# silencht/SG-SLAM

Hardware: AMD Instinct MI355X
Metric: tracked frames/sec (640x480 RGB-D) (higher is better)
Workload: dtype u8/f32(bf16x3 matrix products)/f64

## Files before the change

### include/sgx_debug.h

```cpp
#ifndef SGX_DEBUG_H
#define SGX_DEBUG_H
#include "sgx.h"
#ifdef __cplusplus
extern "C" {
#endif

int sgx_orb_debug_level_geometry(const sgx_orb *h, int level, int32_t *w, int32_t *hgt, int32_t *stride);
int sgx_orb_debug_set_unfused_pyramid(int on);
int sgx_orb_debug_read_level(sgx_orb *h, int frame, int level, uint8_t *dst );
int sgx_orb_debug_read_candidates(sgx_orb *h, int frame, int level, int32_t *x, int32_t *y, int32_t *score, int cap, int *n);
int sgx_debug_flow_affine_batch_dev(int batch, int cap, const sgx_keypoint *d_keys, const int32_t *d_n, const float *d_A, const float *d_shift, const float *d_boxes,
                                    int max_boxes, float *d_prev_xy, void *stream);
int sgx_pose_opt_debug_set_threads(int threads_per_frame);
int sgx_ba_debug_last_plan(int32_t plan[4]);
int sgx_ba_debug_set_init(int mode);
int sgx_ba_debug_set_jobs(int host);
int sgx_ba_debug_set_solver(int mode);
int sgx_det_debug_read_blob(sgx_det *h, const char *blob_name, int image, float *dst, int cap, int *n);
int sgx_flow_debug_read_level(sgx_flow *h, int slot, int frame, int level, uint8_t *img);
int sgx_flow_debug_level_size(const sgx_flow *h, int level, int32_t *w, int32_t *hgt);
int sgx_pnp_debug_betas(int which, const double *L, const double *rho, double *betas);
int sgx_debug_corun_bf16(int blocks, int iters, int launches, void *stream);
int sgx_det_debug_detection_output(sgx_det *h, const float *loc, const float *conf, int batch, sgx_det_result *results);
int sgx_det_debug_continued(sgx_det *h, int *count);
int sgx_det_debug_set_fusion(int on);
int sgx_det_debug_set_irb(int on);
int sgx_det_debug_set_block_fusion(int on);
int sgx_det_debug_set_gemm(int mode);
int sgx_det_debug_set_legacy_kernels(int on);
int sgx_det_debug_time_ops(sgx_det *h, const uint8_t *d_img, int pitch, int batch, int reps, float *ms, int cap, int *nops);
int sgx_det_debug_run_step(sgx_det *h, const uint8_t *d_img, int pitch, int batch, int step, int reps, void *stream);
int sgx_orb_debug_run_octree(sgx_orb *h, int level, const uint32_t *packed, int n, uint32_t *out_sel, int cap, int *nsel);

#ifdef __cplusplus
}
#endif
#endif
```

### sg_slam_amd/capi.py

```python
import ctypes as C
import numpy as np

KP_DTYPE = np.dtype([('x', 'f4'), ('y', 'f4'), ('size', 'f4'), ('angle', 'f4'), ('response', 'f4'),
                     ('octave', 'i4'), ('class_id', 'i4')])


class SgxError(RuntimeError):
    pass


class Camera(C.Structure):
    _fields_ = [('fx', C.c_float), ('fy', C.c_float), ('cx', C.c_float), ('cy', C.c_float), ('bf', C.c_float),
                ('min_x', C.c_float), ('max_x', C.c_float), ('min_y', C.c_float), ('max_y', C.c_float)]


class BaProblem(C.Structure):
    _fields_ = [('n_poses', C.c_int32), ('n_points', C.c_int32), ('n_edges', C.c_int32), ('poses', C.c_void_p), ('pose_fixed', C.c_void_p),
                ('points', C.c_void_p), ('edge_pose', C.c_void_p), ('edge_point', C.c_void_p), ('edge_obs', C.c_void_p), ('edge_info', C.c_void_p)]


class BaStats(C.Structure):
    _fields_ = [('iterations_first', C.c_int32), ('iterations_second', C.c_int32), ('free_poses', C.c_int32), ('reserved', C.c_int32),
                ('chi2_first', C.c_double), ('chi2_second', C.c_double)]


SGX_DET_MAX = 100


class Detection(C.Structure):
    _fields_ = [(k, C.c_float) for k in ('label', 'score', 'xmin', 'ymin', 'xmax', 'ymax')]


class Object2D(C.Structure):
    _fields_ = [('id', C.c_int32)] + [(k, C.c_float) for k in ('prob', 'x', 'y', 'w', 'h')]


class DetResult(C.Structure):
    _fields_ = [('n_raw', C.c_int32), ('raw', Detection * SGX_DET_MAX), ('n_objects', C.c_int32), ('objects', Object2D * SGX_DET_MAX),
                ('have_dynamic_for_mapping', C.c_int32), ('have_dynamic_for_rm_feature', C.c_int32),
                ('n_map_boxes', C.c_int32), ('map_boxes', Object2D * SGX_DET_MAX), ('n_rm_boxes', C.c_int32), ('rm_boxes', Object2D * SGX_DET_MAX)]


class FlowConfig(C.Structure):
    _fields_ = [('width', C.c_int32), ('height', C.c_int32), ('max_batch', C.c_int32), ('win_size', C.c_int32), ('max_level', C.c_int32),
                ('max_count', C.c_int32), ('epsilon', C.c_double)]


class TrackerConfig(C.Structure):
    _fields_ = [('streams', C.c_int32), ('width', C.c_int32), ('height', C.c_int32), ('nfeatures', C.c_int32), ('scale_factor', C.c_float), ('nlevels', C.c_int32),
                ('ini_th_fast', C.c_int32), ('min_th_fast', C.c_int32), ('cam', Camera), ('depth_map_factor', C.c_float), ('th_projection', C.c_float),
                ('local_map', C.c_int32), ('dynamic_mask', C.c_int32), ('max_boxes', C.c_int32), ('pipelined', C.c_int32)]


class OrbConfig(C.Structure):
    _fields_ = [('nfeatures', C.c_int32), ('scale_factor', C.c_float), ('nlevels', C.c_int32),
                ('ini_th_fast', C.c_int32), ('min_th_fast', C.c_int32), ('width', C.c_int32),
                ('height', C.c_int32), ('max_batch', C.c_int32)]


SYMBOLS = [
    'sgx_version', 'sgx_status_string', 'sgx_orb_create', 'sgx_orb_destroy', 'sgx_orb_keypoint_capacity', 'sgx_orb_get_tables',
    'sgx_orb_extract_batch_dev', 'sgx_orb_extract', 'sgx_orb_last_status', 'sgx_profile_enable', 'sgx_profile_num_classes', 'sgx_profile_class_name',
    'sgx_profile_read', 'sgx_match_project_frame_batch_dev', 'sgx_match_project_frame', 'sgx_match_project_local_batch_dev',
    'sgx_match_project_local', 'sgx_frame_stereo_from_rgbd_batch_dev', 'sgx_frame_unproject_batch_dev', 'sgx_frame_make_map_points_batch_dev',
    'sgx_frame_merge_matches_batch_dev', 'sgx_pose_optimization_batch_dev', 'sgx_pose_optimization', 'sgx_frame_motion_model_batch_dev',
    'sgx_local_bundle_adjustment', 'sgx_bundle_adjustment', 'sgx_det_create', 'sgx_det_destroy', 'sgx_det_info', 'sgx_det_detect',
    'sgx_det_detect_batch_dev', 'sgx_det_forward_batch_dev', 'sgx_frame_compact_keys_batch_dev', 'sgx_frame_gray_from_color_batch_dev',
    'sgx_det_gemm_mode', 'sgx_det_plan_step', 'sgx_dynamic_mask_batch_dev', 'sgx_tracker_create', 'sgx_tracker_destroy',
    'sgx_tracker_keypoint_capacity', 'sgx_tracker_record_bytes', 'sgx_tracker_set_initial_pose', 'sgx_tracker_step_dev', 'sgx_tracker_host_buffers',
    'sgx_tracker_step_host', 'sgx_tracker_wait_inputs', 'sgx_tracker_sync', 'sgx_tracker_read', 'sgx_tracker_snapshot_pose_dev',
    'sgx_tracker_snapshot_boxes_dev', 'sgx_tracker_pack_records_dev', 'sgx_tracker_frame_dev', 'sgx_tracker_extractor', 'sgx_flow_create',
    'sgx_dist_unique_id', 'sgx_dist_create', 'sgx_dist_destroy', 'sgx_dist_world', 'sgx_dist_gather_records',
    'sgx_flow_destroy', 'sgx_flow_reset', 'sgx_flow_levels', 'sgx_flow_lk_batch_dev', 'sgx_flow_lk', 'sgx_fundamental_ransac_batch_dev',
    'sgx_find_fundamental_mat', 'sgx_hamming_matrix', 'sgx_hamming_matrix_dev', 'sgx_match_search_for_triangulation', 'sgx_match_search_by_bow',
    'sgx_match_search_by_bow_kf', 'sgx_match_fuse_search', 'sgx_match_project_keyframe', 'sgx_match_fuse_search_sim3',
    'sgx_triangulate_new_map_points', 'sgx_mappoint_update_normal_and_depth', 'sgx_mappoint_distinctive_descriptors', 'sgx_sim3_solver_create',
    'sgx_sim3_solver_set_ransac_parameters', 'sgx_sim3_solver_iterate', 'sgx_sim3_solver_get_estimate', 'sgx_sim3_solver_destroy',
    'sgx_match_search_for_initialization', 'sgx_voc_load', 'sgx_voc_create', 'sgx_voc_info', 'sgx_voc_destroy', 'sgx_voc_transform',
    'sgx_voc_transform_batch_dev', 'sgx_voc_score', 'sgx_match_project_sim3', 'sgx_match_search_by_sim3', 'sgx_optimize_sim3',
    'sgx_optimize_essential_graph', 'sgx_correct_map_points', 'sgx_undistort_points', 'sgx_frame_undistort_stereo_rgbd_batch_dev', 'sgx_frame_image_bounds',
    'sgx_tracker_set_distortion', 'sgx_tracker_frame_keys_un_dev', 'sgx_pnp_solver_create', 'sgx_pnp_solver_set_ransac_parameters', 'sgx_pnp_solver_iterate',
    'sgx_pnp_solver_get_estimate', 'sgx_pnp_solver_destroy', 'sgx_pnp_batch_create', 'sgx_pnp_batch_set_dev', 'sgx_pnp_batch_iterate_dev', 'sgx_pnp_batch_destroy',
]
TAP_SYMBOLS = [
    'sgx_orb_debug_level_geometry', 'sgx_orb_debug_set_unfused_pyramid', 'sgx_orb_debug_read_level', 'sgx_orb_debug_read_candidates',
    'sgx_orb_debug_run_octree', 'sgx_pose_opt_debug_set_threads', 'sgx_ba_debug_set_solver', 'sgx_ba_debug_set_jobs', 'sgx_ba_debug_set_init', 'sgx_ba_debug_last_plan', 'sgx_det_debug_read_blob',
    'sgx_det_debug_detection_output', 'sgx_det_debug_continued', 'sgx_debug_flow_affine_batch_dev', 'sgx_det_debug_set_fusion', 'sgx_det_debug_set_legacy_kernels',
    'sgx_det_debug_set_block_fusion', 'sgx_det_debug_set_irb', 'sgx_det_debug_set_gemm', 'sgx_det_debug_time_ops', 'sgx_det_debug_run_step', 'sgx_flow_debug_read_level',
    'sgx_flow_debug_level_size', 'sgx_debug_corun_bf16', 'sgx_pnp_debug_betas',
]


def _vp(x):
    if x is None:
        return None
    if isinstance(x, int):
        return C.c_void_p(x)
    if hasattr(x, 'data_ptr'):
        return C.c_void_p(x.data_ptr())
    return x.ctypes.data_as(C.c_void_p)


class SgxLib:
    def __init__(self, path):
        self.path = path
        self.dll = C.CDLL(path)
        d = self.dll
        d.sgx_version.restype = C.c_char_p
        d.sgx_status_string.restype = C.c_char_p
        d.sgx_status_string.argtypes = [C.c_int]
        d.sgx_orb_create.argtypes = [C.POINTER(OrbConfig), C.POINTER(C.c_void_p)]
        d.sgx_orb_destroy.argtypes = [C.c_void_p]
        d.sgx_orb_destroy.restype = None
        d.sgx_orb_keypoint_capacity.argtypes = [C.c_void_p]
        d.sgx_orb_get_tables.argtypes = [C.c_void_p] + [C.c_void_p] * 5
        d.sgx_orb_extract_batch_dev.argtypes = [C.c_void_p, C.c_void_p, C.c_int, C.c_int, C.c_void_p, C.c_void_p,
                                                C.c_void_p, C.c_int, C.c_void_p]
        d.sgx_orb_extract.argtypes = [C.c_void_p, C.c_void_p, C.c_int, C.c_void_p, C.c_void_p, C.c_int, C.POINTER(C.c_int)]
        d.sgx_orb_last_status.argtypes = [C.c_void_p, C.c_void_p]

        d.sgx_profile_enable.argtypes = [C.c_int]
        d.sgx_profile_class_name.restype = C.c_char_p
        d.sgx_profile_class_name.argtypes = [C.c_int]
        d.sgx_profile_read.argtypes = [C.c_void_p, C.c_void_p, C.c_int]

        vp = C.c_void_p
        d.sgx_match_project_frame_batch_dev.argtypes = [C.c_int, C.c_int] + [vp] * 13 + [C.POINTER(Camera), vp, C.c_int, C.c_float, C.c_int, C.c_int, vp, vp, vp]
        d.sgx_match_project_frame.argtypes = [C.c_int] + [vp] * 4 + [C.c_int] + [vp] * 7 + [C.POINTER(Camera), vp, C.c_int, C.c_float, C.c_int, C.c_int, vp, vp]
        d.sgx_frame_stereo_from_rgbd_batch_dev.argtypes = [C.c_int, C.c_int, vp, vp, vp, C.c_int, C.c_int, C.c_float, C.c_float, vp, vp, vp]
        d.sgx_frame_unproject_batch_dev.argtypes = [C.c_int, C.c_int, vp, vp, vp, vp, C.POINTER(Camera), vp, vp, vp]
        d.sgx_pose_optimization_batch_dev.argtypes = [C.c_int, C.c_int, vp, vp, vp, vp, vp, vp, C.c_int, vp, C.c_int, C.POINTER(Camera), vp, vp, vp, vp]
        d.sgx_pose_optimization.argtypes = [C.c_int, vp, vp, vp, vp, vp, C.c_int, C.POINTER(Camera), vp, vp, vp]
        d.sgx_frame_motion_model_batch_dev.argtypes = [C.c_int, vp, vp, vp, vp, vp]
        d.sgx_local_bundle_adjustment.argtypes = [C.POINTER(BaProblem), C.POINTER(Camera), vp, vp, C.POINTER(BaStats)]
        d.sgx_bundle_adjustment.argtypes = [C.POINTER(BaProblem), C.POINTER(Camera), C.c_int, vp, C.c_int, C.POINTER(BaStats)]
        d.sgx_det_create.argtypes = [C.c_char_p, vp, C.c_size_t, C.c_int, C.c_int, C.c_int, C.c_float, C.c_float, C.POINTER(vp)]
        d.sgx_det_destroy.argtypes = [vp]; d.sgx_det_destroy.restype = None
        d.sgx_det_info.argtypes = [vp, C.POINTER(C.c_int32), C.POINTER(C.c_int32), C.POINTER(C.c_int32), C.POINTER(C.c_double)]
        d.sgx_det_detect.argtypes = [vp, vp, C.c_int, C.c_int, C.POINTER(DetResult)]
        d.sgx_det_detect_batch_dev.argtypes = [vp, vp, C.c_int, C.c_int, vp, vp, vp, C.c_int, vp, vp]
        d.sgx_det_forward_batch_dev.argtypes = [vp, vp, C.c_int, C.c_int, C.POINTER(vp), C.POINTER(vp), vp]
        d.sgx_det_gemm_mode.argtypes = [vp]
        d.sgx_tracker_create.argtypes = [C.POINTER(TrackerConfig), vp, C.POINTER(vp)]
        d.sgx_tracker_destroy.argtypes = [vp]; d.sgx_tracker_destroy.restype = None
        d.sgx_tracker_keypoint_capacity.argtypes = [vp]
        d.sgx_tracker_record_bytes.argtypes = [vp]
        d.sgx_tracker_set_initial_pose.argtypes = [vp, vp]
        d.sgx_tracker_step_dev.argtypes = [vp, vp, C.c_int, vp, vp, C.c_int, vp]
        d.sgx_tracker_host_buffers.argtypes = [vp, C.c_int, C.POINTER(vp), C.POINTER(C.c_int), C.POINTER(vp)]
        d.sgx_tracker_step_host.argtypes = [vp, C.c_int, C.c_int]
        d.sgx_tracker_sync.argtypes = [vp]
        d.sgx_tracker_wait_inputs.argtypes = [vp, C.c_int]
        d.sgx_tracker_read.argtypes = [vp] * 10
        d.sgx_tracker_snapshot_pose_dev.argtypes = [vp, vp]
        d.sgx_tracker_snapshot_boxes_dev.argtypes = [vp, C.c_int, vp, vp]
        d.sgx_tracker_pack_records_dev.argtypes = [vp, vp, vp]
        d.sgx_dist_unique_id.argtypes = [vp]
        d.sgx_dist_create.argtypes = [vp, C.c_int, C.c_int, C.POINTER(vp)]
        d.sgx_dist_destroy.argtypes = [vp]; d.sgx_dist_destroy.restype = None
        d.sgx_dist_world.argtypes = [vp, C.POINTER(C.c_int32), C.POINTER(C.c_int32)]
        d.sgx_dist_gather_records.argtypes = [vp, vp, C.c_size_t, vp, C.c_int, vp]
        d.sgx_tracker_frame_dev.argtypes = [vp] + [C.POINTER(vp)] * 6
        d.sgx_tracker_extractor.argtypes = [vp]; d.sgx_tracker_extractor.restype = vp
        d.sgx_det_plan_step.argtypes = [vp, C.c_int, C.c_char_p, C.c_int]
        d.sgx_dynamic_mask_batch_dev.argtypes = [C.c_int, C.c_int, vp, vp, vp, vp, vp, vp, C.c_int, vp, vp]
        d.sgx_frame_gray_from_color_batch_dev.argtypes = [C.c_int, C.c_int, C.c_int, vp, C.c_int, C.c_int, C.c_int, vp, C.c_int, vp]
        d.sgx_frame_compact_keys_batch_dev.argtypes = [C.c_int, C.c_int, vp, vp, vp, vp, vp, C.c_int, vp, vp, vp, vp]
        d.sgx_match_project_local.argtypes = [C.c_int] + [vp] * 5 + [C.c_int] + [vp] * 7 + [C.POINTER(Camera), vp, C.c_int, C.c_float, C.c_float, C.c_float, C.c_float, vp, vp, vp]
        d.sgx_match_project_local_batch_dev.argtypes = [C.c_int, C.c_int] + [vp] * 6 + [C.c_int] + [vp] * 8 + [C.POINTER(Camera), vp, C.c_int, C.c_float, C.c_float, C.c_float, C.c_float, vp, vp, vp, vp]
        d.sgx_undistort_points.argtypes = [C.c_int, vp, vp, vp, C.c_int, vp]
        d.sgx_frame_undistort_stereo_rgbd_batch_dev.argtypes = [C.c_int, C.c_int, vp, vp, vp, C.c_int, C.POINTER(Camera), vp, C.c_int, C.c_int, C.c_float, vp, vp, vp, vp]
        d.sgx_frame_image_bounds.argtypes = [C.c_int, C.c_int, vp, vp, C.c_int, C.POINTER(Camera)]
        d.sgx_tracker_set_distortion.argtypes = [vp, vp, C.c_int, C.POINTER(Camera)]
        d.sgx_tracker_frame_keys_un_dev.argtypes = [vp, C.POINTER(vp)]
        d.sgx_frame_make_map_points_batch_dev.argtypes = [C.c_int, C.c_int, C.c_int] + [vp] * 7 + [C.c_int] + [vp] * 7
        d.sgx_frame_merge_matches_batch_dev.argtypes = [C.c_int, C.c_int] + [vp] * 10
        d.sgx_flow_create.argtypes = [C.POINTER(FlowConfig), C.POINTER(vp)]
        d.sgx_flow_destroy.argtypes = [vp]; d.sgx_flow_destroy.restype = None
        d.sgx_flow_reset.argtypes = [vp]
        d.sgx_flow_levels.argtypes = [vp]
        d.sgx_flow_lk_batch_dev.argtypes = [vp, vp, C.c_int, C.c_int, vp, vp, C.c_int, vp, vp, C.POINTER(C.c_int32), vp]
        d.sgx_flow_lk.argtypes = [vp, vp, vp, C.c_int, vp, C.c_int, vp, vp]
        d.sgx_fundamental_ransac_batch_dev.argtypes = [C.c_int, C.c_int] + [vp] * 6 + [C.c_int, C.c_double, C.c_double, vp, vp, vp, vp]
        d.sgx_find_fundamental_mat.argtypes = [vp, vp, C.c_int, C.c_double, C.c_double, vp, vp, vp]
        d.sgx_hamming_matrix.argtypes = [vp, C.c_int, vp, C.c_int, vp]
        d.sgx_optimize_essential_graph.argtypes = [C.c_int, vp, vp, C.c_int, vp, vp, vp, C.c_int, C.c_int, vp, vp]
        d.sgx_correct_map_points.argtypes = [C.c_int, vp, vp, C.c_int, vp, vp, vp]
        d.sgx_optimize_sim3.argtypes = [C.c_int] + [vp] * 9 + [C.c_float, C.c_int, vp, vp, vp]
        d.sgx_match_project_keyframe.argtypes = [C.c_int] + [vp] * 4 + [C.c_int] + [vp] * 6 + [C.POINTER(Camera), vp, C.c_int, C.c_float, C.c_float, C.c_int, C.c_int, vp, vp]
        d.sgx_match_search_by_bow.argtypes = [C.c_int] + [vp] * 4 + [C.c_int] + [vp] * 3 + [C.c_float, C.c_int, vp, vp]
        d.sgx_match_fuse_search_sim3.argtypes = [C.c_int, vp, vp, vp, C.c_int] + [vp] * 6 + [vp, vp, C.c_int, C.c_float, C.c_float, vp, vp, vp]
        d.sgx_match_project_sim3.argtypes = [C.c_int, vp, vp, vp, vp, C.c_int] + [vp] * 6 + [vp, vp, C.c_int, C.c_float, C.c_int, vp, vp]
        d.sgx_match_search_by_sim3.argtypes = ([C.c_int] + [vp] * 8) * 2 + [vp, vp, C.c_int, C.c_float, C.c_float, vp, vp, C.c_float, vp, vp]
        d.sgx_match_search_for_initialization.argtypes = [C.c_int, vp, vp, C.c_int, vp, vp, vp, C.c_int, C.c_float, C.c_int, vp, vp, vp]
        d.sgx_sim3_solver_create.argtypes = [C.c_int] + [vp] * 6 + [C.c_int, C.c_uint, vp]
        d.sgx_sim3_solver_set_ransac_parameters.argtypes = [vp, C.c_double, C.c_int, C.c_int]
        d.sgx_sim3_solver_iterate.argtypes = [vp, C.c_int] + [vp] * 7
        d.sgx_sim3_solver_get_estimate.argtypes = [vp] * 5
        d.sgx_sim3_solver_destroy.argtypes = [vp]; d.sgx_sim3_solver_destroy.restype = None
        d.sgx_pnp_solver_create.argtypes = [C.c_int] + [vp] * 4 + [C.c_uint, vp]
        d.sgx_pnp_solver_set_ransac_parameters.argtypes = [vp, C.c_double, C.c_int, C.c_int, C.c_int, C.c_float, C.c_float]
        d.sgx_pnp_solver_iterate.argtypes = [vp, C.c_int] + [vp] * 7
        d.sgx_pnp_solver_get_estimate.argtypes = [vp] * 6
        d.sgx_pnp_solver_destroy.argtypes = [vp]; d.sgx_pnp_solver_destroy.restype = None
        d.sgx_pnp_batch_create.argtypes = [C.c_int, C.c_int, vp]
        d.sgx_pnp_batch_set_dev.argtypes = [vp, C.c_int] + [vp] * 8
        d.sgx_pnp_batch_iterate_dev.argtypes = [vp, C.c_int, vp, C.c_int, vp, vp, vp, vp]
        d.sgx_pnp_batch_destroy.argtypes = [vp]; d.sgx_pnp_batch_destroy.restype = None
        d.sgx_mappoint_update_normal_and_depth.argtypes = [C.c_int] + [vp] * 6 + [C.c_int, vp, vp, vp]
        d.sgx_mappoint_distinctive_descriptors.argtypes = [C.c_int, vp, vp, vp, vp]
        d.sgx_triangulate_new_map_points.argtypes = [C.c_int, vp] + [C.c_int] + [vp] * 5 + [C.c_int] + [vp] * 5 + [vp, vp, vp, C.c_int, vp, vp, vp]
        d.sgx_voc_load.argtypes = [C.c_char_p, vp]
        d.sgx_voc_create.argtypes = [C.c_int] * 5 + [vp] * 5
        d.sgx_voc_info.argtypes = [vp] * 7
        d.sgx_voc_destroy.argtypes = [vp]; d.sgx_voc_destroy.restype = None
        d.sgx_voc_transform.argtypes = [vp, C.c_int, vp, C.c_int, vp, vp, vp, vp, vp]
        d.sgx_voc_transform_batch_dev.argtypes = [vp, vp, C.c_size_t, vp, C.c_int, C.c_int, C.c_int, vp, vp, vp, vp]
        d.sgx_voc_score.argtypes = [vp, C.c_int, vp, vp, C.c_int, vp, vp, vp]
        d.sgx_match_search_by_bow_kf.argtypes = [C.c_int] + [vp] * 4 + [C.c_int] + [vp] * 4 + [C.c_float, C.c_int, vp, vp]
        d.sgx_match_fuse_search.argtypes = [C.c_int] + [vp] * 4 + [C.c_int] + [vp] * 6 + [C.POINTER(Camera), vp, vp, C.c_int, C.c_float, C.c_float, vp, vp, vp]
        d.sgx_hamming_matrix_dev.argtypes = [vp, C.c_int, vp, C.c_int, vp, vp]
        d.sgx_match_search_for_triangulation.argtypes = [C.c_int] + [vp] * 6 + [C.c_int] + [vp] * 6 + [vp, C.POINTER(Camera), vp, vp, C.c_int, C.c_int, C.c_int, vp, vp]

        self.has_taps = hasattr(d, 'sgx_det_debug_read_blob')
        if self.has_taps:
            d.sgx_orb_debug_level_geometry.argtypes = [C.c_void_p, C.c_int] + [C.POINTER(C.c_int32)] * 3
            d.sgx_orb_debug_read_level.argtypes = [C.c_void_p, C.c_int, C.c_int, C.c_void_p]
            d.sgx_orb_debug_read_candidates.argtypes = [C.c_void_p, C.c_int, C.c_int, C.c_void_p, C.c_void_p, C.c_void_p, C.c_int, C.POINTER(C.c_int)]
            d.sgx_orb_debug_run_octree.argtypes = [C.c_void_p, C.c_int, C.c_void_p, C.c_int, C.c_void_p, C.c_int, C.POINTER(C.c_int)]
            d.sgx_orb_debug_set_unfused_pyramid.argtypes = [C.c_int]
            d.sgx_pose_opt_debug_set_threads.argtypes = [C.c_int]
            d.sgx_ba_debug_set_solver.argtypes = [C.c_int]
            d.sgx_ba_debug_set_jobs.argtypes = [C.c_int]
            d.sgx_ba_debug_set_init.argtypes = [C.c_int]
            d.sgx_ba_debug_last_plan.argtypes = [C.c_void_p]
            d.sgx_det_debug_detection_output.argtypes = [vp, vp, vp, C.c_int, C.POINTER(DetResult)]
            d.sgx_det_debug_continued.argtypes = [vp, C.POINTER(C.c_int)]
            d.sgx_det_debug_read_blob.argtypes = [vp, C.c_char_p, C.c_int, vp, C.c_int, C.POINTER(C.c_int)]
            for nm in ('fusion', 'legacy_kernels', 'block_fusion', 'irb', 'gemm'):
                getattr(d, 'sgx_det_debug_set_' + nm).argtypes = [C.c_int]
            d.sgx_det_debug_time_ops.argtypes = [vp, vp, C.c_int, C.c_int, C.c_int, vp, C.c_int, C.POINTER(C.c_int)]
            d.sgx_det_debug_run_step.argtypes = [vp, vp, C.c_int, C.c_int, C.c_int, C.c_int, vp]
            d.sgx_debug_flow_affine_batch_dev.argtypes = [C.c_int, C.c_int, vp, vp, vp, vp, vp, C.c_int, vp, vp]
            d.sgx_flow_debug_read_level.argtypes = [vp, C.c_int, C.c_int, C.c_int, vp]
            d.sgx_debug_corun_bf16.argtypes = [C.c_int, C.c_int, C.c_int, vp]
            d.sgx_pnp_debug_betas.argtypes = [C.c_int, vp, vp, vp]
            d.sgx_flow_debug_level_size.argtypes = [vp, C.c_int, C.POINTER(C.c_int32), C.POINTER(C.c_int32)]

    def tap(self, name):
        if not self.has_taps:
            raise SgxError(f'{name}: {self.path} is the product build and has no test taps; use tests/taps/libsgx_taps.so (make -C sg_slam_amd/csrc taps)')
        return getattr(self.dll, name)

    def version(self):
        return self.dll.sgx_version().decode()

    def check(self, rc, what=''):
        if rc != 0:
            raise SgxError(f'{what}: {self.dll.sgx_status_string(rc).decode()} ({rc})')

    def profile_enable(self, on=True):
        self.check(self.dll.sgx_profile_enable(int(on)))

    def profile_read(self, reset=True):
        n = self.dll.sgx_profile_num_classes()
        ms = np.zeros(n, 'f4'); cnt = np.zeros(n, 'i4')
        self.check(self.dll.sgx_profile_read(_vp(ms), _vp(cnt), int(reset)), 'sgx_profile_read')
        return {self.dll.sgx_profile_class_name(k).decode(): (float(ms[k]), int(cnt[k])) for k in range(n)}
```

### sg_slam_amd/csrc/sgx_flow.cpp

```cpp
#include "sgx_flow_kernels.h"
#include "sgx_prof.h"
#include "sgx_stage.h"
#include "../../include/sgx.h"
#ifdef SGX_DEBUG_TAPS
#include "../../include/sgx_debug.h"
#endif
#include <stdio.h>
#include <stdlib.h>
#include <string.h>
#include <new>
#include <vector>


struct sgx_flow {
    sgx_flow_config cfg;
    SgxLkGeom g;
    uint8_t *img[2] = { nullptr, nullptr };
    int cur = 0;
    int prev_batch = 0;
};

extern "C" int sgx_flow_create(const sgx_flow_config *cfg, sgx_flow **out)
{
    if (!cfg || !out) return SGX_ERR_INVALID;
    *out = nullptr;
    if (cfg->width < 1 || cfg->height < 1 || cfg->max_batch < 1 || cfg->max_count < 0 || !(cfg->epsilon >= 0)) return SGX_ERR_INVALID;
    if (cfg->win_size != SGX_LK_WIN || cfg->max_level < 0 || cfg->max_level >= SGX_LK_MAXL) return SGX_ERR_UNSUPPORTED;
    if (cfg->width <= 1 || cfg->height <= 1) return SGX_ERR_UNSUPPORTED;
    { const unsigned long long qw = (unsigned long long)((cfg->width + 3) >> 2); if (qw * qw * (unsigned long long)cfg->height >= (1ull << 32)) return SGX_ERR_UNSUPPORTED; }
    sgx_flow *h = new (std::nothrow) sgx_flow();
    if (!h) return SGX_ERR_NOMEM;
    h->cfg = *cfg;
    SgxLkGeom &g = h->g;
    memset(&g, 0, sizeof g);
    int w = cfg->width, hh = cfg->height; unsigned io = 0;
    for (int l = 0;; l++) {
        g.w[l] = w; g.h[l] = hh; g.pitch[l] = (w + 3) & ~3; g.ioff[l] = io;
        io += (unsigned)g.pitch[l] * (unsigned)hh;
        g.nl = l + 1;
        if (l == cfg->max_level) break;
        const int nw = (w + 1) / 2, nh = (hh + 1) / 2;
        if (nw <= cfg->win_size || nh <= cfg->win_size) break;
        w = nw; hh = nh;
    }
    g.img_stride = (io + 15u + 64u) & ~15u;
    for (int s = 0; s < 2; s++)
        if (hipMalloc((void **)&h->img[s], (size_t)g.img_stride * cfg->max_batch) != hipSuccess) { sgx_flow_destroy(h); return SGX_ERR_NOMEM; }
    *out = h;
    return SGX_OK;
}

extern "C" void sgx_flow_destroy(sgx_flow *h)
{
    if (!h) return;
    for (int s = 0; s < 2; s++) if (h->img[s]) (void)hipFree(h->img[s]);
    delete h;
}

extern "C" int sgx_flow_reset(sgx_flow *h) { if (!h) return SGX_ERR_INVALID; h->prev_batch = 0; return SGX_OK; }
extern "C" int sgx_flow_levels(const sgx_flow *h) { return h ? h->g.nl : SGX_ERR_INVALID; }

static int build_pyramid(sgx_flow *h, int slot, const uint8_t *d_gray, int pitch, int batch, sgx_stream_t st)
{
    const SgxLkGeom &g = h->g;
    uint8_t *base = h->img[slot];
    sgx_prof_begin(SGX_K_LK_PYR, st);
    auto magic = [](int d) -> unsigned { return d <= 1 ? 0u : (unsigned)((0x100000000ull + (unsigned)d - 1) / (unsigned)d); };
    SGX_LAUNCH(k_lk_copy, dim3(((g.pitch[0] >> 2) * g.h[0] + 255) / 256, batch), dim3(256), st, d_gray, g.w[0], g.h[0], pitch, base, g.pitch[0], g.img_stride, magic(g.pitch[0] >> 2));
    for (int l = 1; l < g.nl; l++)
        SGX_LAUNCH(k_lk_pyrdown, dim3(((g.pitch[l] >> 2) * g.h[l] + 255) / 256, batch), dim3(256), st, (const uint8_t *)(base + g.ioff[l - 1]), g.w[l - 1], g.h[l - 1], g.pitch[l - 1],
                   g.img_stride, base + g.ioff[l], g.w[l], g.h[l], g.pitch[l], g.img_stride, magic(g.pitch[l] >> 2));
    sgx_prof_end(SGX_K_LK_PYR, st);
    SGX_CHECK_HIP(hipGetLastError());
    return SGX_OK;
}

static int track(sgx_flow *h, int cur_slot, int prev_slot, int batch, const sgx_keypoint *d_keys, const int32_t *d_n, int cap, float *d_prev_xy, uint8_t *d_status, sgx_stream_t st)
{
    SgxLkArgs A;
    A.cur_img = h->img[cur_slot]; A.prev_img = h->img[prev_slot];
    A.keys = (const uint8_t *)d_keys; A.n = d_n; A.cap = cap; A.prev_xy = d_prev_xy; A.status = d_status;
    A.max_count = h->cfg.max_count > 100 ? 100 : h->cfg.max_count;
    double eps = h->cfg.epsilon > 10. ? 10. : h->cfg.epsilon;
    A.eps2 = eps * eps; A.min_eig = (float)1e-4;
    sgx_prof_begin(SGX_K_LK_TRACK, st);
    static const int kpw = sgx_getenv("SGX_LK_KPW") ? atoi(sgx_getenv("SGX_LK_KPW")) : 2;
    A.batch = batch; A.kblocks = (cap + 4 * kpw - 1) / (4 * kpw);
#ifdef SGX_DEBUG_TAPS
    if (kpw == 4) { auto kfn = k_lk_trackN<4>; SGX_LAUNCH(kfn, dim3((unsigned)A.kblocks * (unsigned)batch), dim3(256), st, h->g, A); }
    else if (kpw != 2) { A.kblocks = (cap + 3) / 4; SGX_LAUNCH(k_lk_track, dim3((unsigned)A.kblocks * (unsigned)batch), dim3(256), st, h->g, A); }
    else
#endif
    { auto kfn = k_lk_trackN<2>; SGX_LAUNCH(kfn, dim3((unsigned)A.kblocks * (unsigned)batch), dim3(256), st, h->g, A); }
    sgx_prof_end(SGX_K_LK_TRACK, st);
    SGX_CHECK_HIP(hipGetLastError());
    return SGX_OK;
}

extern "C" int sgx_flow_lk_batch_dev(sgx_flow *h, const uint8_t *d_gray, int pitch, int batch, const sgx_keypoint *d_keys, const int32_t *d_n, int cap,
                                     float *d_prev_xy, uint8_t *d_status, int32_t *have_prev, void *stream)
{
    if (!h || !d_gray || batch < 1 || batch > h->cfg.max_batch || pitch < h->cfg.width) return SGX_ERR_INVALID;
    if ((pitch & 3) || ((uintptr_t)d_gray & 3)) return SGX_ERR_INVALID;
    sgx_stream_t st = (sgx_stream_t)stream;
    const int cur = h->cur, prev = cur ^ 1;
    const bool tracked = h->prev_batch == batch;
    if (tracked && (!d_keys || !d_n || !d_prev_xy || cap < 1)) return SGX_ERR_INVALID;
    int rc = build_pyramid(h, cur, d_gray, pitch, batch, st);
    if (rc != SGX_OK) return rc;
    if (tracked) { rc = track(h, cur, prev, batch, d_keys, d_n, cap, d_prev_xy, d_status, st); if (rc != SGX_OK) return rc; }
    if (have_prev) *have_prev = tracked ? 1 : 0;
    h->cur = prev; h->prev_batch = batch;
    return SGX_OK;
}

extern "C" int sgx_flow_lk(sgx_flow *h, const uint8_t *gray_from, const uint8_t *gray_to, int stride, const float *pts, int n, float *next_pts, uint8_t *status)
{
    if (!h || !gray_from || !gray_to || stride < h->cfg.width || n < 0 || (n > 0 && (!pts || !next_pts))) return SGX_ERR_INVALID;
    if (n == 0) return SGX_OK;
    const int W = h->cfg.width, H = h->cfg.height, P = (W + 3) & ~3;
    std::vector<uint8_t> pack((size_t)P * H * 2, 0);
    for (int y = 0; y < H; y++) { memcpy(&pack[(size_t)y * P], gray_to + (size_t)y * stride, (size_t)W); memcpy(&pack[(size_t)(H + y) * P], gray_from + (size_t)y * stride, (size_t)W); }
    std::vector<sgx_keypoint> kp((size_t)n);
    for (int i = 0; i < n; i++) { memset(&kp[(size_t)i], 0, sizeof(sgx_keypoint)); kp[(size_t)i].x = pts[2 * i]; kp[(size_t)i].y = pts[2 * i + 1]; }
    SgxStaged dI, dK, dN, dO, dS;
    int rc;
    if ((rc = dI.put(0, pack.data(), pack.size())) != SGX_OK || (rc = dK.put(1, kp.data(), kp.size() * sizeof(sgx_keypoint))) != SGX_OK ||
        (rc = dN.put(2, &n, sizeof n)) != SGX_OK || (rc = dO.put(3, nullptr, (size_t)n * 8)) != SGX_OK || (rc = dS.put(4, nullptr, (size_t)n)) != SGX_OK) return rc;
    const int keep_cur = h->cur, keep_prev = h->prev_batch;
    if ((rc = build_pyramid(h, 1, (const uint8_t *)dI.p, P, 1, 0)) != SGX_OK) return rc;
    if ((rc = build_pyramid(h, 0, (const uint8_t *)dI.p + (size_t)P * H, P, 1, 0)) != SGX_OK) return rc;
    if ((rc = track(h, 0, 1, 1, (const sgx_keypoint *)dK.p, (const int32_t *)dN.p, n, (float *)dO.p, (uint8_t *)dS.p, 0)) != SGX_OK) return rc;
    SGX_CHECK_HIP(hipMemcpy(next_pts, dO.p, (size_t)n * 8, hipMemcpyDeviceToHost));
    if (status) SGX_CHECK_HIP(hipMemcpy(status, dS.p, (size_t)n, hipMemcpyDeviceToHost));
    h->cur = keep_cur; h->prev_batch = 0; (void)keep_prev;
    return SGX_OK;
}

SGX_TAP int sgx_flow_debug_read_level(sgx_flow *h, int slot, int frame, int level, uint8_t *img )
{
    if (!h || slot < 0 || slot > 1 || frame < 0 || frame >= h->cfg.max_batch || level < 0 || level >= h->g.nl) return SGX_ERR_INVALID;
    const SgxLkGeom &g = h->g;
    SGX_CHECK_HIP(hipDeviceSynchronize());
    if (!img) return SGX_ERR_INVALID;
    {
        std::vector<uint8_t> t((size_t)g.pitch[level] * g.h[level]);
        SGX_CHECK_HIP(hipMemcpy(t.data(), h->img[slot] + (size_t)frame * g.img_stride + g.ioff[level], t.size(), hipMemcpyDeviceToHost));
        for (int y = 0; y < g.h[level]; y++) memcpy(img + (size_t)y * g.w[level], &t[(size_t)y * g.pitch[level]], (size_t)g.w[level]);
    }
    return SGX_OK;
}
SGX_TAP int sgx_flow_debug_level_size(const sgx_flow *h, int level, int32_t *w, int32_t *hh)
{
    if (!h || level < 0 || level >= h->g.nl || !w || !hh) return SGX_ERR_INVALID;
    *w = h->g.w[level]; *hh = h->g.h[level];
    return SGX_OK;
}

#if defined(SGX_DEBUG_TAPS) && !defined(SGX_EMU)
typedef float sgx_dbg_f16v __attribute__((ext_vector_type(16)));
typedef __bf16 sgx_dbg_bf8 __attribute__((ext_vector_type(8)));
SGX_KERNEL_OCC(256, 2) k_dbg_corun_bf16(float *o, int iters)
{
    const uint32_t x = threadIdx.x * 2654435761u + blockIdx.x, y = x ^ 0x9e3779b9u;
    sgx_dbg_f16v acc = {0}; sgx_dbg_bf8 a, b;
    for (int i = 0; i < 8; i++) { a[i] = (__bf16)(float)((x >> i) & 7); b[i] = (__bf16)(float)((y >> i) & 3); }
    for (int i = 0; i < iters; i++) acc = __builtin_amdgcn_mfma_f32_32x32x16_bf16(a, b, acc, 0, 0, 0);
    float s = 0.f; for (int i = 0; i < 16; i++) s += acc[i];
    o[(blockIdx.x & 1023) * 256 + threadIdx.x] = s;
}
#endif
SGX_TAP int sgx_debug_corun_bf16(int blocks, int iters, int launches, void *stream)
{
#if defined(SGX_DEBUG_TAPS) && !defined(SGX_EMU)
    static float *sink = nullptr;
    if (blocks < 1 || iters < 1 || launches < 1) return SGX_ERR_INVALID;
    if (!sink) SGX_CHECK_HIP(hipMalloc((void **)&sink, 1024 * 256 * sizeof(float)));
    for (int l = 0; l < launches; l++) SGX_LAUNCH(k_dbg_corun_bf16, dim3((unsigned)blocks), dim3(256), (sgx_stream_t)stream, sink, iters);
    SGX_CHECK_HIP(hipGetLastError());
    return SGX_OK;
#else
    (void)blocks; (void)iters; (void)launches; (void)stream;
    return SGX_ERR_UNSUPPORTED;
#endif
}

extern "C" int sgx_fundamental_ransac_batch_dev(int batch, int cap, const sgx_keypoint *d_keys, const int32_t *d_n, const float *d_prev_xy,
                                                const int32_t *d_pre_have_dynamic, const float *d_pre_boxes, const int32_t *d_pre_nboxes, int max_boxes,
                                                double threshold, double confidence, double *d_F, int32_t *d_ok, int32_t *d_stats, void *stream)
{
    if (batch < 1 || cap < 1 || !d_keys || !d_n || !d_prev_xy || !d_F || !d_ok || max_boxes < 0) return SGX_ERR_INVALID;
    if (cap > SGX_FM_MAXPTS) return SGX_ERR_UNSUPPORTED;
    SgxFmArgs A;
    A.keys = (const uint8_t *)d_keys; A.n = d_n; A.cap = cap; A.prev_xy = d_prev_xy;
    A.pre_have = d_pre_have_dynamic; A.pre_boxes = d_pre_boxes; A.pre_nboxes = d_pre_nboxes; A.max_boxes = max_boxes;
    if (threshold <= 0) threshold = 3;
    if (confidence < DBL_EPSILON || confidence > 1 - DBL_EPSILON) confidence = 0.99;
    A.threshold = threshold; A.confidence = confidence; A.max_iters = 1000;
    A.F = d_F; A.ok = d_ok; A.stats = d_stats;
    const size_t lds = (size_t)cap * 16 + 1024 + (((size_t)cap + 15) & ~(size_t)15);
    sgx_prof_begin(SGX_K_FM_RANSAC, (sgx_stream_t)stream);
    SGX_LAUNCH_DYN(k_fm_ransac, dim3(batch), dim3(256), lds, (sgx_stream_t)stream, A);
    sgx_prof_end(SGX_K_FM_RANSAC, (sgx_stream_t)stream);
    SGX_CHECK_HIP(hipGetLastError());
    return SGX_OK;
}

extern "C" int sgx_find_fundamental_mat(const float *pts1, const float *pts2, int n, double threshold, double confidence, double *F, int32_t *ok, int32_t *stats)
{
    if (n < 0 || (n > 0 && (!pts1 || !pts2)) || !F || !ok) return SGX_ERR_INVALID;
    if (n > SGX_FM_MAXPTS) return SGX_ERR_UNSUPPORTED;
    const int cap = n > 0 ? n : 1;
    std::vector<sgx_keypoint> kp((size_t)cap);
    memset(kp.data(), 0, kp.size() * sizeof(sgx_keypoint));
    for (int i = 0; i < n; i++) { kp[(size_t)i].x = pts1[2 * i]; kp[(size_t)i].y = pts1[2 * i + 1]; }
    SgxStaged dK, dN, dP, dF, dO, dS;
    int rc;
    if ((rc = dK.put(0, kp.data(), kp.size() * sizeof(sgx_keypoint))) != SGX_OK || (rc = dN.put(1, &n, sizeof n)) != SGX_OK ||
        (rc = dP.put(2, n ? pts2 : nullptr, (size_t)cap * 8)) != SGX_OK || (rc = dF.put(3, nullptr, 72)) != SGX_OK || (rc = dO.put(4, nullptr, 4)) != SGX_OK ||
        (rc = dS.put(5, nullptr, 16)) != SGX_OK) return rc;
    rc = sgx_fundamental_ransac_batch_dev(1, cap, (const sgx_keypoint *)dK.p, (const int32_t *)dN.p, (const float *)dP.p, nullptr, nullptr, nullptr, 0, threshold, confidence,
                                          (double *)dF.p, (int32_t *)dO.p, (int32_t *)dS.p, nullptr);
    if (rc != SGX_OK) return rc;
    SGX_CHECK_HIP(hipMemcpy(F, dF.p, 72, hipMemcpyDeviceToHost));
    SGX_CHECK_HIP(hipMemcpy(ok, dO.p, 4, hipMemcpyDeviceToHost));
    if (stats) SGX_CHECK_HIP(hipMemcpy(stats, dS.p, 16, hipMemcpyDeviceToHost));
    return SGX_OK;
}
```

### sg_slam_amd/csrc/sgx_flow_kernels.h

```cpp
#pragma once
#include "sgx_rt.h"
#include "sgx_block.h"
#include <float.h>
#include <math.h>

#define SGX_LK_MAXL 4
#define SGX_LK_WIN 21
#define SGX_LK_TILE_PITCH 36
struct SgxLkGeom {
    int nl;
    int w[SGX_LK_MAXL], h[SGX_LK_MAXL], pitch[SGX_LK_MAXL];
    unsigned ioff[SGX_LK_MAXL];
    unsigned img_stride;
};

SGX_DEV int sgx_reflect101(int p, int len)
{
    if (len == 1) return 0;
    while (p < 0 || p >= len) { if (p < 0) p = -p; else p = 2 * len - 2 - p; }
    return p;
}
SGX_DEV int sgx_floor_f(float v) { return (int)floorf(v); }
SGX_DEV float sgx_i64_to_f32(long long v)
{
    const long long hi = v >> 24; const int lo = (int)(v - (hi << 24));
    return (float)(int)hi * 16777216.0f + (float)lo;
}

SGX_DEV unsigned sgx_lk_udiv(unsigned n, unsigned m)
{
#ifndef SGX_EMU
    return m ? __umulhi(n, m) : n;
#else
    return m ? (unsigned)(((unsigned long long)n * m) >> 32) : n;
#endif
}
SGX_KERNEL(256) k_lk_copy(const uint8_t *src, int w, int h, int spitch, uint8_t *dst, int dpitch, unsigned dstride, unsigned qw_magic)
{
    SGX_THREADS_BEGIN(tid)
    const int f = (int)blockIdx.y, qw = dpitch >> 2, q = (int)blockIdx.x * 256 + tid;
    if (q < qw * h) {
        const int y = (int)sgx_lk_udiv((unsigned)q, qw_magic), x = (q - y * qw) * 4;
        const uint8_t *s = src + ((size_t)f * h + y) * spitch;
        uint32_t v;
        if (x + 4 <= w) v = *(const uint32_t *)(s + x);
        else { v = 0; for (int i = 0; x + i < w; i++) v |= (uint32_t)s[x + i] << (8 * i); }
        *(uint32_t *)(dst + (size_t)f * dstride + (size_t)y * dpitch + x) = v;
    }
    SGX_THREADS_END
}

SGX_KERNEL(256) k_lk_pyrdown(const uint8_t *src, int sw, int sh, int spitch, unsigned sstride, uint8_t *dst, int dw, int dh, int dpitch, unsigned dstride, unsigned qw_magic)
{
    SGX_THREADS_BEGIN(tid)
    const int f = (int)blockIdx.y, qw = dpitch >> 2, q = (int)blockIdx.x * 256 + tid;
    if (q < qw * dh) {
        const int y = (int)sgx_lk_udiv((unsigned)q, qw_magic), X = (q - y * qw) * 4;
        const uint8_t *S = src + (size_t)f * sstride;
        int acc[4] = { 0, 0, 0, 0 };
        const bool fast = X >= 2 && 2 * X + 11 < spitch && 2 * X + 8 <= sw - 1;
#pragma unroll
        for (int k = 0; k < 5; k++) {
            const int wk = k == 0 || k == 4 ? 1 : k == 2 ? 6 : 4;
            const uint8_t *row = S + (size_t)sgx_reflect101(2 * y - 2 + k, sh) * spitch;
            int p[11];
            if (fast) {
                const uint32_t *r4 = (const uint32_t *)(row + 2 * X - 4);
                const uint32_t a = r4[0], b = r4[1], c = r4[2], d = r4[3];
                p[0] = (a >> 16) & 255; p[1] = a >> 24;
                p[2] = b & 255; p[3] = (b >> 8) & 255; p[4] = (b >> 16) & 255; p[5] = b >> 24;
                p[6] = c & 255; p[7] = (c >> 8) & 255; p[8] = (c >> 16) & 255; p[9] = c >> 24;
                p[10] = d & 255;
            } else {
#pragma unroll
                for (int i = 0; i < 11; i++) p[i] = row[sgx_reflect101(2 * X - 2 + i, sw)];
            }
#pragma unroll
            for (int o = 0; o < 4; o++) acc[o] += wk * (p[2 * o + 2] * 6 + (p[2 * o + 1] + p[2 * o + 3]) * 4 + p[2 * o] + p[2 * o + 4]);
        }
        uint32_t out = 0;
#pragma unroll
        for (int o = 0; o < 4; o++) out |= (uint32_t)((acc[o] + 128) >> 8) << (8 * o);
        *(uint32_t *)(dst + (size_t)f * dstride + (size_t)y * dpitch + X) = out;
    }
    SGX_THREADS_END
}

struct SgxLkWeights { int w00, w01, w10, w11; };
SGX_DEV SgxLkWeights sgx_lk_weights(float a, float b)
{
    SgxLkWeights k;
    k.w00 = sgx_cvround((1.f - a) * (1.f - b) * (float)(1 << 14));
    k.w01 = sgx_cvround(a * (1.f - b) * (float)(1 << 14));
    k.w10 = sgx_cvround((1.f - a) * b * (float)(1 << 14));
    k.w11 = (1 << 14) - k.w00 - k.w01 - k.w10;
    return k;
}
#define SGX_LK_DESCALE(x, n) (((x) + (1 << ((n) - 1))) >> (n))

struct SgxLkStep { float dx, dy; };
SGX_DEV SgxLkStep sgx_lk_step(float A11, float A12, float A22, float D, long long sb1, long long sb2)
{
    const float FLT_SCALE = 1.f / (1 << 20);
    const float b1 = sgx_i64_to_f32(sb1) * FLT_SCALE, b2 = sgx_i64_to_f32(sb2) * FLT_SCALE;
    SgxLkStep s;
    s.dx = (A12 * b2 - A22 * b1) * D;
    s.dy = (A12 * b1 - A11 * b2) * D;
    return s;
}

struct SgxLkArgs {
    const uint8_t *cur_img, *prev_img;
    const uint8_t *keys; const int *n; int cap;
    float *prev_xy; uint8_t *status;
    int max_count; double eps2; float min_eig;
    int batch, kblocks;
};
SGX_DEV void sgx_lk_decode_block(int i, int batch, int kblocks, int &f, int &kb)
{
    const int full = (batch / 8) * 8;
    if (i < full * kblocks) { const int x = i & 7, j = i >> 3; kb = j % kblocks; f = x + 8 * (j / kblocks); }
    else { const int j = i - full * kblocks; f = full + j / kblocks; kb = j % kblocks; }
}

#ifdef SGX_EMU
static inline int sgx_lk_px(const uint8_t *I, int w, int h, int pitch, int x, int y) { return I[(size_t)sgx_reflect101(y, h) * pitch + sgx_reflect101(x, w)]; }
static void sgx_lk_track_point(const SgxLkGeom &g, const uint8_t *I0, const uint8_t *J0, float kx, float ky, int max_count, double eps2, float min_eig,
                               float *ox, float *oy, uint8_t *ost)
{
    const int W = SGX_LK_WIN; const float half = (W - 1) * 0.5f, FLT_SCALE = 1.f / (1 << 20);
    float outx = 0.f, outy = 0.f; uint8_t status = 1;
    static thread_local short Iw[SGX_LK_WIN * SGX_LK_WIN], dIw[SGX_LK_WIN * SGX_LK_WIN * 2];
    for (int level = g.nl - 1; level >= 0; level--) {
        const int w = g.w[level], h = g.h[level], pitch = g.pitch[level];
        const uint8_t *I = I0 + g.ioff[level], *J = J0 + g.ioff[level];
        const float sc = 1.0f / (float)(1 << level);
        float prevx = kx * sc, prevy = ky * sc, nextx, nexty;
        if (level == g.nl - 1) { nextx = prevx; nexty = prevy; } else { nextx = outx * 2.f; nexty = outy * 2.f; }
        outx = nextx; outy = nexty;
        prevx -= half; prevy -= half;
        const int ipx = sgx_floor_f(prevx), ipy = sgx_floor_f(prevy);
        if (ipx < -W || ipx >= w || ipy < -W || ipy >= h) { if (level == 0) status = 0; continue; }
        SgxLkWeights k = sgx_lk_weights(prevx - ipx, prevy - ipy);
        long long s11 = 0, s12 = 0, s22 = 0;
        for (int y = 0; y < W; y++) for (int x = 0; x < W; x++) {
            int pv[4], dx[4], dy[4];
            for (int c = 0; c < 4; c++) {
                const int gx = ipx + x + (c & 1), gy = ipy + y + (c >> 1);
                pv[c] = sgx_lk_px(I, w, h, pitch, gx, gy);
                if (gx < 0 || gy < 0 || gx >= w || gy >= h) { dx[c] = dy[c] = 0; }
                else {
                    int t0[3], t1[3];
                    for (int q = 0; q < 3; q++) {
                        const int a = sgx_lk_px(I, w, h, pitch, gx - 1 + q, gy - 1), b = sgx_lk_px(I, w, h, pitch, gx - 1 + q, gy), cc = sgx_lk_px(I, w, h, pitch, gx - 1 + q, gy + 1);
                        t0[q] = (a + cc) * 3 + b * 10; t1[q] = cc - a;
                    }
                    dx[c] = t0[2] - t0[0]; dy[c] = (t1[0] + t1[2]) * 3 + t1[1] * 10;
                }
            }
            const int iv = SGX_LK_DESCALE(pv[0] * k.w00 + pv[1] * k.w01 + pv[2] * k.w10 + pv[3] * k.w11, 9);
            const int ix = SGX_LK_DESCALE(dx[0] * k.w00 + dx[1] * k.w01 + dx[2] * k.w10 + dx[3] * k.w11, 14);
            const int iy = SGX_LK_DESCALE(dy[0] * k.w00 + dy[1] * k.w01 + dy[2] * k.w10 + dy[3] * k.w11, 14);
            Iw[y * W + x] = (short)iv; dIw[(y * W + x) * 2] = (short)ix; dIw[(y * W + x) * 2 + 1] = (short)iy;
            s11 += (long long)ix * ix; s12 += (long long)ix * iy; s22 += (long long)iy * iy;
        }
        const float A11 = sgx_i64_to_f32(s11) * FLT_SCALE, A12 = sgx_i64_to_f32(s12) * FLT_SCALE, A22 = sgx_i64_to_f32(s22) * FLT_SCALE;
        float D = A11 * A22 - A12 * A12;
        const float minEig = (A22 + A11 - sqrtf((A11 - A22) * (A11 - A22) + 4.f * A12 * A12)) / (float)(2 * W * W);
        if (minEig < min_eig || D < FLT_EPSILON) { if (level == 0) status = 0; continue; }
        D = 1.f / D;
        nextx -= half; nexty -= half;
        float pdx = 0.f, pdy = 0.f;
        for (int j = 0; j < max_count; j++) {
            const int inx = sgx_floor_f(nextx), iny = sgx_floor_f(nexty);
            if (inx < -W || inx >= w || iny < -W || iny >= h) { if (level == 0) status = 0; break; }
            k = sgx_lk_weights(nextx - inx, nexty - iny);
            long long sb1 = 0, sb2 = 0;
            for (int y = 0; y < W; y++) for (int x = 0; x < W; x++) {
                int pv[4];
                for (int c = 0; c < 4; c++) pv[c] = sgx_lk_px(J, w, h, pitch, inx + x + (c & 1), iny + y + (c >> 1));
                const int diff = SGX_LK_DESCALE(pv[0] * k.w00 + pv[1] * k.w01 + pv[2] * k.w10 + pv[3] * k.w11, 9) - Iw[y * W + x];
                sb1 += (long long)diff * dIw[(y * W + x) * 2]; sb2 += (long long)diff * dIw[(y * W + x) * 2 + 1];
            }
            const SgxLkStep st = sgx_lk_step(A11, A12, A22, D, sb1, sb2);
            nextx += st.dx; nexty += st.dy;
            outx = nextx + half; outy = nexty + half;
            if ((double)st.dx * st.dx + (double)st.dy * st.dy <= eps2) break;
            if (j > 0 && fabs((double)(st.dx + pdx)) < 0.01 && fabs((double)(st.dy + pdy)) < 0.01) { outx -= st.dx * 0.5f; outy -= st.dy * 0.5f; break; }
            pdx = st.dx; pdy = st.dy;
        }
        if (status && level == 0) {
            const int ix = sgx_floor_f(outx - half), iy = sgx_floor_f(outy - half);
            if (ix < -W || ix >= w || iy < -W || iy >= h) status = 0;
        }
    }
    *ox = outx; *oy = outy; *ost = status;
}
SGX_KERNEL(256) k_lk_track(SgxLkGeom g, SgxLkArgs A)
{
    SGX_THREADS_BEGIN(tid)
    int f, kb;
    sgx_lk_decode_block((int)blockIdx.x, A.batch, A.kblocks, f, kb);
    const int kp = kb * 4 + (tid >> 6);
    if ((tid & 63) == 0 && kp < A.n[f] && kp < A.cap) {
        const float *kpt = (const float *)(A.keys + ((size_t)f * A.cap + kp) * 28);
        float ox, oy; uint8_t st;
        sgx_lk_track_point(g, A.cur_img + (size_t)f * g.img_stride, A.prev_img + (size_t)f * g.img_stride, kpt[0], kpt[1], A.max_count, A.eps2, A.min_eig, &ox, &oy, &st);
        A.prev_xy[2 * ((size_t)f * A.cap + kp)] = ox; A.prev_xy[2 * ((size_t)f * A.cap + kp) + 1] = oy;
        if (A.status) A.status[(size_t)f * A.cap + kp] = st;
    }
    SGX_THREADS_END
}
#else
SGX_DEV int sgx_wave_sum_i32(int v)
{
    v += __builtin_amdgcn_update_dpp(0, v, 0xB1, 0xF, 0xF, true);
    v += __builtin_amdgcn_update_dpp(0, v, 0x4E, 0xF, 0xF, true);
    v += __builtin_amdgcn_update_dpp(0, v, 0x124, 0xF, 0xF, true);
    v += __builtin_amdgcn_update_dpp(0, v, 0x128, 0xF, 0xF, true);
    v += __builtin_amdgcn_update_dpp(0, v, 0x142, 0xA, 0xF, false);
    v += __builtin_amdgcn_update_dpp(0, v, 0x143, 0xC, 0xF, false);
    return __builtin_amdgcn_readlane(v, 63);
}
SGX_DEV float sgx_wave_sum_f32(int v)
{
    const int lo = sgx_wave_sum_i32(v & 0xFFFF), hi = sgx_wave_sum_i32(v >> 16);
    return fmaf((float)hi, 65536.0f, (float)lo);
}
SGX_DEV int sgx_mul24(int a, int b) { return __mul24(a, b); }
SGX_DEV int sgx_reflect1(int p, int len) { p = p < 0 ? -p : p; p = p >= len ? 2 * len - 2 - p : p; return min(max(p, 0), len - 1); }

typedef short sgx_i16x2 __attribute__((ext_vector_type(2)));
typedef unsigned short sgx_u16x2 __attribute__((ext_vector_type(2)));
SGX_DEV sgx_i16x2 sgx_as_i16x2(uint32_t v) { return __builtin_bit_cast(sgx_i16x2, v); }
SGX_DEV uint32_t sgx_as_u32(sgx_i16x2 v) { return __builtin_bit_cast(uint32_t, v); }
#define SGX_LK_PAIR(hi, lo, a, b) sgx_as_i16x2(__builtin_amdgcn_perm((hi), (lo), (uint32_t)(a) | 0x0c00u | ((uint32_t)(b) << 16) | 0x0c000000u))
SGX_DEV sgx_i16x2 sgx_lk_next(sgx_i16x2 p, sgx_i16x2 q) { return sgx_as_i16x2(__builtin_amdgcn_alignbit(sgx_as_u32(q), sgx_as_u32(p), 16)); }
#if defined(SGX_LK_NODOT) && !defined(SGX_EMU)
SGX_DEV int sgx_lk_dot2_mad(sgx_i16x2 a, sgx_i16x2 b, int c)
{
    const uint32_t ua = __builtin_bit_cast(uint32_t, a), ub = __builtin_bit_cast(uint32_t, b);
    asm("v_mad_i32_i16 %0, %1, %2, %0 op_sel:[0,0,0,0]" : "+v"(c) : "v"(ua), "v"(ub));
    asm("v_mad_i32_i16 %0, %1, %2, %0 op_sel:[1,1,0,0]" : "+v"(c) : "v"(ua), "v"(ub));
    return c;
}
#define SGX_LK_DOT2(a, b, c) sgx_lk_dot2_mad((a), (b), (c))
#else
#define SGX_LK_DOT2(a, b, c) __builtin_amdgcn_sdot2((a), (b), (c), false)
#endif
SGX_DEV int sgx_lk_dot2_keep(sgx_i16x2 a, sgx_i16x2 b, int c) { return SGX_LK_DOT2(a, b, c); }

template <int PASSES>
SGX_DEV void sgx_lk_stage(uint32_t *tile, const uint8_t *img, int w, int h, int pitch, int ox, int oy, int rl, int cl)
{
    __builtin_amdgcn_fence(__ATOMIC_SEQ_CST, "wavefront"); __builtin_amdgcn_wave_barrier();
    const int gx = ox + 4 * cl;
    const bool inside = gx >= 0 && gx + 4 <= w;
    if (rl < 7) {
        uint32_t v[PASSES];
        if (inside) {
#pragma unroll
            for (int p = 0; p < PASSES; p++) v[p] = *(const uint32_t *)(img + (size_t)sgx_reflect1(oy + p * 7 + rl, h) * pitch + gx);
        } else {
            const int x0 = sgx_reflect1(gx, w), x1 = sgx_reflect1(gx + 1, w), x2 = sgx_reflect1(gx + 2, w), x3 = sgx_reflect1(gx + 3, w);
#pragma unroll
            for (int p = 0; p < PASSES; p++) {
                const uint8_t *src = img + (size_t)sgx_reflect1(oy + p * 7 + rl, h) * pitch;
                v[p] = (uint32_t)src[x0] | ((uint32_t)src[x1] << 8) | ((uint32_t)src[x2] << 16) | ((uint32_t)src[x3] << 24);
            }
        }
#pragma unroll
        for (int p = 0; p < PASSES; p++) tile[(p * 7 + rl) * (SGX_LK_TILE_PITCH / 4) + cl] = v[p];
    }
    __builtin_amdgcn_fence(__ATOMIC_SEQ_CST, "wavefront"); __builtin_amdgcn_wave_barrier();
}

#ifdef SGX_DEBUG_TAPS
SGX_KERNEL(256) k_lk_track(SgxLkGeom g, SgxLkArgs A)
{
    __shared__ uint32_t tiles[4][35 * SGX_LK_TILE_PITCH / 4 + 5];
    const int tid = (int)threadIdx.x, lane = tid & 63, wv = tid >> 6;
    int f, kb;
    sgx_lk_decode_block((int)blockIdx.x, A.batch, A.kblocks, f, kb);
    const int kp = kb * 4 + wv;
    if (kp >= A.n[f] || kp >= A.cap) return;
    uint32_t *tile = tiles[wv];
    const uint8_t *tile8 = (const uint8_t *)tile;
    const int W = SGX_LK_WIN; const float half = 10.0f, FLT_SCALE = 1.f / (1 << 20);
    const float *kpt = (const float *)(A.keys + ((size_t)f * A.cap + kp) * 28);
    const float kx = __builtin_bit_cast(float, __builtin_amdgcn_readfirstlane(__builtin_bit_cast(int, kpt[0])));
    const float ky = __builtin_bit_cast(float, __builtin_amdgcn_readfirstlane(__builtin_bit_cast(int, kpt[1])));
    const uint8_t *I0 = A.cur_img + (size_t)f * g.img_stride, *J0 = A.prev_img + (size_t)f * g.img_stride;
    const int r = lane / 3, s7 = (lane - 3 * r) * 7;
    const int rl = lane / 9, cl = lane - 9 * rl;
    const bool active = lane < 63;
    const int lane_off = active ? r * SGX_LK_TILE_PITCH + s7 : 0;
    float outx = 0.f, outy = 0.f; int status = 1;

    for (int level = g.nl - 1; level >= 0; level--) {
        const int w = g.w[level], h = g.h[level], pitch = g.pitch[level];
        const uint8_t *I = I0 + g.ioff[level], *J = J0 + g.ioff[level];
        const float sc = 1.0f / (float)(1 << level);
        float prevx = kx * sc, prevy = ky * sc, nextx, nexty;
        if (level == g.nl - 1) { nextx = prevx; nexty = prevy; } else { nextx = outx * 2.f; nexty = outy * 2.f; }
        outx = nextx; outy = nexty;
        prevx -= half; prevy -= half;
        const int ipx = sgx_floor_f(prevx), ipy = sgx_floor_f(prevy);
        if (ipx < -W || ipx >= w || ipy < -W || ipy >= h) { if (level == 0) status = 0; continue; }
        SgxLkWeights k = sgx_lk_weights(prevx - ipx, prevy - ipy);
        sgx_i16x2 W0 = sgx_as_i16x2((uint32_t)k.w00 | ((uint32_t)k.w01 << 16)), W1 = sgx_as_i16x2((uint32_t)k.w10 | ((uint32_t)k.w11 << 16));

        int ivb[7]; int ix[7], iy[7];
        int s11 = 0, s12 = 0, s22 = 0;
        {
            const int gy0 = ipy + r, gx0 = ipx + s7;
            sgx_i16x2 P[4][5];
            const bool direct = ipx >= 1 && ipx + 25 < w && ipy >= 1 && ipy + 22 < h;
            if (direct) {
                const uint8_t *gb = I + (size_t)(active ? gy0 - 1 : ipy) * pitch + (active ? gx0 - 1 : ipx);
#pragma unroll
                for (int j = 0; j < 4; j++) {
                    uint32_t q[3];
                    __builtin_memcpy(q, gb + (size_t)j * pitch, 12);
                    P[j][0] = SGX_LK_PAIR(q[0], q[0], 0, 1); P[j][1] = SGX_LK_PAIR(q[0], q[0], 2, 3);
                    P[j][2] = SGX_LK_PAIR(q[1], q[1], 0, 1); P[j][3] = SGX_LK_PAIR(q[1], q[1], 2, 3);
                    P[j][4] = SGX_LK_PAIR(q[2], q[2], 0, 1);
                }
            } else {
                const int tx = ((ipx - 1) >> 2) << 2, ty = ipy - 1;
                sgx_lk_stage<4>(tile, I, w, h, pitch, tx, ty, rl, cl);
                const uint8_t *tb = tile8 + lane_off + (ipx - 1 - tx);
#pragma unroll
                for (int j = 0; j < 4; j++) {
                    uint32_t q[3];
                    __builtin_memcpy(q, tb + j * SGX_LK_TILE_PITCH, 12);
                    P[j][0] = SGX_LK_PAIR(q[0], q[0], 0, 1); P[j][1] = SGX_LK_PAIR(q[0], q[0], 2, 3);
                    P[j][2] = SGX_LK_PAIR(q[1], q[1], 0, 1); P[j][3] = SGX_LK_PAIR(q[1], q[1], 2, 3);
                    P[j][4] = SGX_LK_PAIR(q[2], q[2], 0, 1);
                }
            }
            const sgx_i16x2 c3 = { 3, 3 }, c10 = { 10, 10 };
            const sgx_i16x2 Wd0 = active ? W0 : sgx_as_i16x2(0u), Wd1 = active ? W1 : sgx_as_i16x2(0u);
            sgx_i16x2 S0[5], S1[5], D0[5], D1[5];
#pragma unroll
            for (int q = 0; q < 5; q++) {
                S0[q] = (P[0][q] + P[2][q]) * c3 + P[1][q] * c10; D0[q] = P[2][q] - P[0][q];
                S1[q] = (P[1][q] + P[3][q]) * c3 + P[2][q] * c10; D1[q] = P[3][q] - P[1][q];
            }
            sgx_i16x2 xa[5], ya[5], xb[5], yb[5];
            const bool whole = ipx >= 0 && ipx + W < w && ipy >= 0 && ipy + W < h;
#pragma unroll
            for (int q = 0; q < 4; q++) {
                xa[q] = S0[q + 1] - S0[q]; ya[q] = (D0[q] + D0[q + 1]) * c3 + sgx_lk_next(D0[q], D0[q + 1]) * c10;
                xb[q] = S1[q + 1] - S1[q]; yb[q] = (D1[q] + D1[q + 1]) * c3 + sgx_lk_next(D1[q], D1[q + 1]) * c10;
            }
            if (!whole) {
                const bool rowa = gy0 >= 0 && gy0 < h, rowb = gy0 + 1 >= 0 && gy0 + 1 < h;
#pragma unroll
                for (int q = 0; q < 4; q++) {
                    const int x = gx0 + 2 * q;
                    const uint32_t m = ((x >= 0 && x < w) ? 0xFFFFu : 0u) | ((x + 1 >= 0 && x + 1 < w) ? 0xFFFF0000u : 0u);
                    const uint32_t ma = rowa ? m : 0u, mb = rowb ? m : 0u;
                    xa[q] = sgx_as_i16x2(sgx_as_u32(xa[q]) & ma); ya[q] = sgx_as_i16x2(sgx_as_u32(ya[q]) & ma);
                    xb[q] = sgx_as_i16x2(sgx_as_u32(xb[q]) & mb); yb[q] = sgx_as_i16x2(sgx_as_u32(yb[q]) & mb);
                }
            }
#pragma unroll
            for (int c = 0; c < 7; c++) {
                const sgx_i16x2 pxa = (c & 1) ? sgx_lk_next(xa[c >> 1], xa[(c >> 1) + 1]) : xa[c >> 1], pxb = (c & 1) ? sgx_lk_next(xb[c >> 1], xb[(c >> 1) + 1]) : xb[c >> 1];
                const sgx_i16x2 pya = (c & 1) ? sgx_lk_next(ya[c >> 1], ya[(c >> 1) + 1]) : ya[c >> 1], pyb = (c & 1) ? sgx_lk_next(yb[c >> 1], yb[(c >> 1) + 1]) : yb[c >> 1];
                const sgx_i16x2 pia = (c & 1) ? P[1][(c + 1) >> 1] : sgx_lk_next(P[1][c >> 1], P[1][(c >> 1) + 1]), pib = (c & 1) ? P[2][(c + 1) >> 1] : sgx_lk_next(P[2][c >> 1], P[2][(c >> 1) + 1]);
                const int v = SGX_LK_DOT2(pib, W1, SGX_LK_DOT2(pia, W0, 256)) >> 9;
                const int vx = SGX_LK_DOT2(pxb, Wd1, SGX_LK_DOT2(pxa, Wd0, 8192)) >> 14;
                const int vy = SGX_LK_DOT2(pyb, Wd1, SGX_LK_DOT2(pya, Wd0, 8192)) >> 14;
                ivb[c] = 256 - (v << 9); ix[c] = vx; iy[c] = vy;
                s11 += sgx_mul24(vx, vx); s12 += sgx_mul24(vx, vy); s22 += sgx_mul24(vy, vy);
            }
        }
        const float A11 = sgx_wave_sum_f32(s11) * FLT_SCALE, A12 = sgx_wave_sum_f32(s12) * FLT_SCALE, A22 = sgx_wave_sum_f32(s22) * FLT_SCALE;
        float D = A11 * A22 - A12 * A12;
        const float minEig = (A22 + A11 - sqrtf((A11 - A22) * (A11 - A22) + 4.f * A12 * A12)) / (float)(2 * W * W);
        if (minEig < A.min_eig || D < FLT_EPSILON) { if (level == 0) status = 0; continue; }
        D = 1.f / D;
        nextx -= half; nexty -= half;
        float pdx = 0.f, pdy = 0.f;
        int ox = 0, oy = 0; bool staged = false;
        for (int j = 0; j < A.max_count; j++) {
            const int inx = sgx_floor_f(nextx), iny = sgx_floor_f(nexty);
// ... 665 lines not shown
```

### sg_slam_amd/csrc/sgx_orb.cpp

```cpp
#include "sgx_orb_kernels.h"
#include "sgx_prof.h"
#include "../../include/sgx.h"
#ifdef SGX_DEBUG_TAPS
#include "../../include/sgx_debug.h"
#endif
#include "../../include/sgx_orb_pattern.h"
#include <math.h>
#include <stdio.h>
#include <stdlib.h>
#include <string.h>
#include <vector>

#ifdef SGX_EMU
thread_local sgx_dim3 blockIdx, blockDim, gridDim;
#endif


struct sgx_orb {
    sgx_orb_config cfg;
    SgxOrbGeom g;
    float scale[SGX_MAX_LEVELS], inv_scale[SGX_MAX_LEVELS], sigma2[SGX_MAX_LEVELS], inv_sigma2[SGX_MAX_LEVELS];
    int umax_h[16];
    SgxCell *d_cells = nullptr;
    SgxXTab *d_xt[SGX_MAX_LEVELS] = {};
    SgxYTab *d_yt[SGX_MAX_LEVELS] = {};
    SgxXTab *d_xt_all = nullptr; SgxYTab *d_yt_all = nullptr; SgxPyrRect *d_pyr_rects = nullptr; SgxPyrTabs pyr_tabs; int pyr_tiles = 0, pyr_lds = 0;
    int *d_umax = nullptr;
    signed char *d_pattern = nullptr;
    uint8_t *d_pyr = nullptr;
    uint8_t *d_blur = nullptr; SgxBlurTile *d_blur_tiles = nullptr;
    uint32_t *d_cand = nullptr;
    int *d_cand_count = nullptr;
    uint16_t *d_node_scratch = nullptr;
    uint32_t *d_sel = nullptr;
    int *d_sel_count = nullptr;
    uint32_t *d_status = nullptr;
    uint8_t *d_gray1 = nullptr; uint8_t *d_kps1 = nullptr; uint8_t *d_desc1 = nullptr; int *d_count1 = nullptr;
    int last_batch = 0;
    int oct_maxlim = 0;
};

static thread_local int g_orb_unfused_pyramid = 0;
SGX_TAP int sgx_orb_debug_set_unfused_pyramid(int on) { g_orb_unfused_pyramid = on ? 1 : 0; return SGX_OK; }

static inline int cvround_f(float v) { return (int)lrintf(v); }
static inline int cvround_d(double v) { return (int)lrint(v); }

static void build_tables(sgx_orb *h)
{
    const sgx_orb_config &c = h->cfg;
    const double sf = (double)c.scale_factor;
    const int nl = c.nlevels;
    h->scale[0] = 1.0f; h->sigma2[0] = 1.0f;
    for (int i = 1; i < nl; i++) { h->scale[i] = (float)((double)h->scale[i - 1] * sf); h->sigma2[i] = h->scale[i] * h->scale[i]; }
    for (int i = 0; i < nl; i++) { h->inv_scale[i] = 1.0f / h->scale[i]; h->inv_sigma2[i] = 1.0f / h->sigma2[i]; }
    const float factor = (float)(1.0f / sf);
    float want = c.nfeatures * (1 - factor) / (1 - (float)pow((double)factor, (double)nl));
    int sum = 0;
    for (int l = 0; l < nl - 1; l++) { h->g.lv[l].quota = cvround_f(want); sum += h->g.lv[l].quota; want *= factor; }
    h->g.lv[nl - 1].quota = c.nfeatures - sum > 0 ? c.nfeatures - sum : 0;
    int umax[17] = {0};
    const int HP = 15;
    const int vmax = (int)floor(HP * sqrtf(2.f) / 2 + 1), vmin = (int)ceil(HP * sqrtf(2.f) / 2);
    for (int v = 0; v <= vmax; ++v) umax[v] = cvround_d(sqrt((double)HP * HP - v * v));
    for (int v = HP, v0 = 0; v >= vmin; --v) { while (umax[v0] == umax[v0 + 1]) ++v0; umax[v] = v0; ++v0; }
    for (int i = 0; i < 16; i++) h->umax_h[i] = umax[i];
}

static void build_resize_tables(int sw, int sh, int dw, int dh, std::vector<SgxXTab> &xt, std::vector<SgxYTab> &yt)
{
    const double scale_x = 1. / ((double)dw / sw), scale_y = 1. / ((double)dh / sh);
    xt.resize(dw); yt.resize(dh);
    for (int dx = 0; dx < dw; dx++) {
        float fx = (float)((dx + 0.5) * scale_x - 0.5);
        int sx = (int)floorf(fx);
        fx -= sx;
        if (sx < 0) { fx = 0; sx = 0; }
        if (sx >= sw - 1) { fx = 0; sx = sw - 1; }
        xt[dx].sx = (short)sx; xt[dx].sx1 = (short)(sx + 1 < sw ? sx + 1 : sx);
        xt[dx].a0 = (short)cvround_f((1.f - fx) * 2048); xt[dx].a1 = (short)cvround_f(fx * 2048);
    }
    for (int dy = 0; dy < dh; dy++) {
        float fy = (float)((dy + 0.5) * scale_y - 0.5);
        int sy = (int)floorf(fy);
        fy -= sy;
        int r0 = sy, r1 = sy + 1;
        if (r0 < 0) r0 = 0; if (r0 > sh - 1) r0 = sh - 1;
        if (r1 < 0) r1 = 0; if (r1 > sh - 1) r1 = sh - 1;
        yt[dy].sy0 = (short)r0; yt[dy].sy1 = (short)r1;
        yt[dy].b0 = (short)cvround_f((1.f - fy) * 2048); yt[dy].b1 = (short)cvround_f(fy * 2048);
    }
}

extern "C" const char *sgx_version(void) {
#ifdef SGX_EMU
    return "sgx 0.1 (EMULATOR - tests only)";
#else
    return "sgx 0.1 (gfx950)";
#endif
}

extern "C" const char *sgx_status_string(int s)
{
    switch (s) {
    case SGX_OK: return "ok";
    case SGX_ERR_INVALID: return "invalid argument";
    case SGX_ERR_UNSUPPORTED: return "unsupported geometry";
    case SGX_ERR_NOMEM: return "out of memory";
    case SGX_ERR_DEVICE: return "HIP runtime error";
    case SGX_ERR_OVERFLOW: return "device buffer overflow";
    default: return "unknown";
    }
}

extern "C" void sgx_orb_destroy(sgx_orb *h)
{
    if (!h) return;
    (void)hipFree(h->d_cells); (void)hipFree(h->d_umax); (void)hipFree(h->d_pattern); (void)hipFree(h->d_pyr); (void)hipFree(h->d_cand);
    (void)hipFree(h->d_cand_count); (void)hipFree(h->d_node_scratch); (void)hipFree(h->d_sel); (void)hipFree(h->d_sel_count); (void)hipFree(h->d_status);
    (void)hipFree(h->d_gray1); (void)hipFree(h->d_kps1); (void)hipFree(h->d_desc1); (void)hipFree(h->d_count1);
    for (int l = 0; l < SGX_MAX_LEVELS; l++) { (void)hipFree(h->d_xt[l]); (void)hipFree(h->d_yt[l]); }
    (void)hipFree(h->d_xt_all); (void)hipFree(h->d_yt_all); (void)hipFree(h->d_pyr_rects); (void)hipFree(h->d_blur); (void)hipFree(h->d_blur_tiles);
    delete h;
}

extern "C" int sgx_orb_create(const sgx_orb_config *cfg, sgx_orb **out)
{
    if (!cfg || !out) return SGX_ERR_INVALID;
    if (cfg->nlevels < 1 || cfg->nlevels > SGX_MAX_LEVELS || cfg->nfeatures < 1 || cfg->width < 64 || cfg->height < 64 ||
        cfg->width > 4000 || cfg->height > 4000 || cfg->max_batch < 1 || !(cfg->scale_factor > 1.0f)) return SGX_ERR_INVALID;
    sgx_orb *h = new sgx_orb();
    h->cfg = *cfg;
    SgxOrbGeom &g = h->g;
    memset(&g, 0, sizeof g);
    g.nlevels = cfg->nlevels; g.W = cfg->width; g.H = cfg->height; g.ini_th = cfg->ini_th_fast; g.min_th = cfg->min_th_fast;
    build_tables(h);
    std::vector<SgxCell> cells;
    int off = 0, kp_cap = 0, cand_off = 0;
    for (int l = 0; l < g.nlevels; l++) {
        SgxLevel &L = g.lv[l];
        L.w = cvround_f((float)cfg->width * h->inv_scale[l]);
        L.h = cvround_f((float)cfg->height * h->inv_scale[l]);
        L.stride = (L.w + 63) & ~63;
        L.scale = h->scale[l];
        L.patch_size = (int)(31 * h->scale[l]);
        if (l > 0) { L.off = off; off += L.stride * L.h; }
        if (L.w < 2 * SGX_EDGE + 8 || L.h < 2 * SGX_EDGE + 8) { sgx_orb_destroy(h); return SGX_ERR_UNSUPPORTED; }
        const float W = 30;
        const int minBX = SGX_BORDER, minBY = SGX_BORDER, maxBX = L.w - SGX_EDGE + 3, maxBY = L.h - SGX_EDGE + 3;
        const float width = (float)(maxBX - minBX), height = (float)(maxBY - minBY);
        L.ncols = (int)(width / W); L.nrows = (int)(height / W);
        if (L.ncols < 1 || L.nrows < 1) { sgx_orb_destroy(h); return SGX_ERR_UNSUPPORTED; }
        L.wcell = (int)ceilf(width / L.ncols); L.hcell = (int)ceilf(height / L.nrows);
        L.cell0 = (int)cells.size();
        L.cand_off = cand_off; L.cand_cap = 0;
        if (L.wcell + 6 > SGX_TILE_MAX || L.hcell + 6 > SGX_TILE_MAX || L.ncols > 1023 || L.nrows > 1023 || L.wcell > 1023 || L.hcell > 1023) {
            sgx_orb_destroy(h); return SGX_ERR_UNSUPPORTED; }
        for (int i = 0; i < L.nrows; i++) {
            const float iniY = (float)(minBY + i * L.hcell);
            float maxY = iniY + L.hcell + 6;
            if (iniY >= maxBY - 3) continue;
            if (maxY > maxBY) maxY = (float)maxBY;
            for (int j = 0; j < L.ncols; j++) {
                const float iniX = (float)(minBX + j * L.wcell);
                float maxX = iniX + L.wcell + 6;
                if (iniX >= maxBX - 6) continue;
                if (maxX > maxBX) maxX = (float)maxBX;
                SgxCell c; c.level = (short)l; c.x0 = (short)iniX; c.y0 = (short)iniY;
                c.cw = (short)((int)maxX - (int)iniX); c.ch = (short)((int)maxY - (int)iniY);
                c.ox = (short)(j * L.wcell); c.oy = (short)(i * L.hcell);
                { const int ng = ((c.x0 & 3) + c.cw + 3) >> 2; c.pad = (short)(unsigned short)((65536 + ng - 1) / ng); }
                if (c.cw >= 7 && c.ch >= 7) {
                    cells.push_back(c);
                    L.cand_cap += ((c.cw - 6 + 1) / 2) * ((c.ch - 6 + 1) / 2);
                }
            }
        }
        const int nIni = (int)roundf((float)(maxBX - minBX) / (float)(maxBY - minBY));
        if (nIni < 1 || nIni > 64) { sgx_orb_destroy(h); return SGX_ERR_UNSUPPORTED; }
        int lim = L.quota + 3; if (lim < 4 * nIni) lim = 4 * nIni;
        if (lim > SGX_OCT_MAXN) { sgx_orb_destroy(h); return SGX_ERR_UNSUPPORTED; }
        kp_cap += lim;
        if (lim > h->oct_maxlim) h->oct_maxlim = lim;
        L.cand_cap = (L.cand_cap + 63) & ~63;
        cand_off += L.cand_cap;
    }
    g.cand_pitch = cand_off;
    {
        int mw = 7, mh = 7;
        for (const SgxCell &cc : cells) { if (cc.cw > mw) mw = cc.cw; if (cc.ch > mh) mh = cc.ch; }
        const int tile_b = mh * SGX_TILE_STRIDE, q_b = ((mw - 6) * (mh - 6) * 2 + 15) & ~15, o_b = (((mw - 5) / 2) * ((mh - 5) / 2) * 4 + 15) & ~15;
        g.fast_off_score = tile_b; g.fast_off_qlist = 2 * tile_b; g.fast_off_out = 2 * tile_b + q_b; g.fast_lds_bytes = 2 * tile_b + q_b + o_b;
    }
    g.pyr_pitch = (off + 255) & ~255;
    std::vector<SgxBlurTile> btiles;
    {
        int boff = 0;
        for (int l = 0; l < g.nlevels; l++) {
            SgxLevel &L = g.lv[l];
            L.bstride = (L.w + 63) & ~63; L.boff = boff; boff += L.bstride * L.h;
            for (int y0 = 0; y0 < L.h; y0 += SGX_BT_H) for (int x0 = 0; x0 < L.w; x0 += SGX_BT_W) {
                SgxBlurTile t; memset(&t, 0, sizeof t);
                t.level = (short)l; t.x0 = (short)x0; t.y0 = (short)y0; t.w = (short)std::min(SGX_BT_W, L.w - x0); t.h = (short)std::min(SGX_BT_H, L.h - y0);
                btiles.push_back(t);
            }
        }
        g.blur_pitch = (boff + 255) & ~255; g.nblur_tiles = (int)btiles.size();
    }
    g.ncells = (int)cells.size();
    g.kp_cap = kp_cap;

    const int B = cfg->max_batch, nl = g.nlevels;
#define SGX_ALLOC(p, bytes) do { if (hipMalloc((void **)&(p), (bytes)) != hipSuccess) { sgx_orb_destroy(h); return SGX_ERR_NOMEM; } } while (0)
    SGX_ALLOC(h->d_cells, cells.size() * sizeof(SgxCell));
    SGX_ALLOC(h->d_umax, 16 * sizeof(int));
    SGX_ALLOC(h->d_pattern, 1024);
    SGX_ALLOC(h->d_pyr, (size_t)B * g.pyr_pitch + 256);
    SGX_ALLOC(h->d_blur, (size_t)B * g.blur_pitch + 256);
    SGX_ALLOC(h->d_blur_tiles, btiles.size() * sizeof(SgxBlurTile));
    SGX_CHECK_HIP(hipMemcpy(h->d_blur_tiles, btiles.data(), btiles.size() * sizeof(SgxBlurTile), hipMemcpyHostToDevice));
    SGX_ALLOC(h->d_cand, (size_t)B * g.cand_pitch * 4);
    SGX_ALLOC(h->d_node_scratch, (size_t)B * g.cand_pitch * 2);
    SGX_ALLOC(h->d_cand_count, (size_t)B * nl * 4);
    SGX_ALLOC(h->d_sel, (size_t)B * nl * SGX_OCT_MAXN * 4);
    SGX_ALLOC(h->d_sel_count, (size_t)B * nl * 4);
    SGX_ALLOC(h->d_status, 4);
    SGX_ALLOC(h->d_gray1, (size_t)((g.W + 3) & ~3) * g.H);
    SGX_ALLOC(h->d_kps1, (size_t)kp_cap * 28);
    SGX_ALLOC(h->d_desc1, (size_t)kp_cap * 32);
    SGX_ALLOC(h->d_count1, 4);
    SGX_CHECK_HIP(hipMemcpyAsync(h->d_cells, cells.data(), cells.size() * sizeof(SgxCell), hipMemcpyHostToDevice, 0));
    SGX_CHECK_HIP(hipMemcpyAsync(h->d_umax, h->umax_h, 16 * sizeof(int), hipMemcpyHostToDevice, 0));
    SGX_CHECK_HIP(hipMemcpyAsync(h->d_pattern, sgx_orb_pattern_xy, 1024, hipMemcpyHostToDevice, 0));
    SGX_CHECK_HIP(hipMemsetAsync(h->d_status, 0, 4, 0));
    for (int l = 1; l < nl; l++) {
        std::vector<SgxXTab> xt; std::vector<SgxYTab> yt;
        build_resize_tables(g.lv[l - 1].w, g.lv[l - 1].h, g.lv[l].w, g.lv[l].h, xt, yt);
        SGX_ALLOC(h->d_xt[l], xt.size() * sizeof(SgxXTab));
        SGX_ALLOC(h->d_yt[l], yt.size() * sizeof(SgxYTab));
        SGX_CHECK_HIP(hipMemcpyAsync(h->d_xt[l], xt.data(), xt.size() * sizeof(SgxXTab), hipMemcpyHostToDevice, 0));
        SGX_CHECK_HIP(hipMemcpyAsync(h->d_yt[l], yt.data(), yt.size() * sizeof(SgxYTab), hipMemcpyHostToDevice, 0));
        SGX_CHECK_HIP(hipStreamSynchronize(0));
    }
    SGX_CHECK_HIP(hipStreamSynchronize(0));
    if (nl > 1) {
        std::vector<std::vector<SgxXTab>> xts(nl); std::vector<std::vector<SgxYTab>> yts(nl);
        std::vector<SgxXTab> xall; std::vector<SgxYTab> yall;
        memset(&h->pyr_tabs, 0, sizeof h->pyr_tabs);
        for (int l = 1; l < nl; l++) {
            build_resize_tables(g.lv[l - 1].w, g.lv[l - 1].h, g.lv[l].w, g.lv[l].h, xts[l], yts[l]);
            h->pyr_tabs.xoff[l] = (int)xall.size(); h->pyr_tabs.yoff[l] = (int)yall.size();
            xall.insert(xall.end(), xts[l].begin(), xts[l].end()); yall.insert(yall.end(), yts[l].begin(), yts[l].end());
        }
        const int T = 32, ntx = (g.lv[nl - 1].w + T - 1) / T, nty = (g.lv[nl - 1].h + T - 1) / T;
        std::vector<SgxPyrRect> rects((size_t)ntx * nty * nl);
        int max_a = 0, max_b = 0, max_x = 0, max_y = 0;
        for (int j = 0; j < nty; j++) for (int i = 0; i < ntx; i++) {
            SgxPyrRect *R = &rects[((size_t)j * ntx + i) * nl];
            int nx0 = 0, nx1 = 0, ny0 = 0, ny1 = 0;
            for (int l = nl - 1; l >= 0; l--) {
                const int Wl = g.lv[l].w, Hl = g.lv[l].h;
                int ax0 = Wl, ax1 = 0, ay0 = Hl, ay1 = 0;
                if (l >= 1) {
                    ax0 = i == 0 ? 0 : (int)(((long)i * Wl / ntx) & ~3L); ax1 = i == ntx - 1 ? Wl : (int)(((long)(i + 1) * Wl / ntx) & ~3L);
                    ay0 = (int)((long)j * Hl / nty); ay1 = j == nty - 1 ? Hl : (int)((long)(j + 1) * Hl / nty);
                }
                SgxPyrRect &r = R[l];
                r.ox0 = (short)ax0; r.ox1 = (short)ax1; r.oy0 = (short)ay0; r.oy1 = (short)ay1;
                if (l < nl - 1) {
                    for (int x = nx0; x < std::min(nx1, g.lv[l + 1].w); x++) { ax0 = std::min(ax0, (int)xts[l + 1][x].sx); ax1 = std::max(ax1, (int)xts[l + 1][x].sx1 + 1); }
                    for (int y = ny0; y < ny1; y++) { ay0 = std::min(ay0, (int)yts[l + 1][y].sy0); ay1 = std::max(ay1, (int)yts[l + 1][y].sy1 + 1); }
                }
                ax0 &= ~3; ax1 = (ax1 + 3) & ~3;
                r.nx0 = (short)ax0; r.ny0 = (short)ay0; r.nw = (short)(ax1 - ax0); r.nh = (short)(ay1 - ay0);
                const int q = r.nw / 4; r.qmagic = q <= 1 ? 0u : (unsigned)((0x100000000ull + (unsigned)q - 1) / (unsigned)q); r.pad = 0;
                const int bytes = (int)r.nw * r.nh;
                if (l & 1) max_b = std::max(max_b, bytes); else max_a = std::max(max_a, bytes);
                nx0 = ax0; nx1 = ax1; ny0 = ay0; ny1 = ay1;
            }
            int xo = 0, yo = 0;
            for (int l = 1; l < nl; l++) { R[l].xo = xo; R[l].yo = yo; xo += R[l].nw; yo += R[l].nh; }
            R[0].xo = R[0].yo = 0;
            max_x = std::max(max_x, xo); max_y = std::max(max_y, yo);
        }
        h->pyr_tabs.lds_a = (max_a + 15) & ~15; h->pyr_tabs.lds_b = (max_b + 15) & ~15; h->pyr_tabs.lds_x = max_x * (int)sizeof(SgxXTab);
        h->pyr_lds = h->pyr_tabs.lds_a + h->pyr_tabs.lds_b + h->pyr_tabs.lds_x + max_y * (int)sizeof(SgxYTab);
        h->pyr_tiles = ntx * nty;
        if (h->pyr_lds > 64 * 1024) h->pyr_tiles = 0;
        SGX_ALLOC(h->d_xt_all, xall.size() * sizeof(SgxXTab)); SGX_ALLOC(h->d_yt_all, yall.size() * sizeof(SgxYTab)); SGX_ALLOC(h->d_pyr_rects, rects.size() * sizeof(SgxPyrRect));
        SGX_CHECK_HIP(hipMemcpy(h->d_xt_all, xall.data(), xall.size() * sizeof(SgxXTab), hipMemcpyHostToDevice));
        SGX_CHECK_HIP(hipMemcpy(h->d_yt_all, yall.data(), yall.size() * sizeof(SgxYTab), hipMemcpyHostToDevice));
        SGX_CHECK_HIP(hipMemcpy(h->d_pyr_rects, rects.data(), rects.size() * sizeof(SgxPyrRect), hipMemcpyHostToDevice));
    }
#undef SGX_ALLOC
    *out = h;
    return SGX_OK;
}

extern "C" int sgx_orb_keypoint_capacity(const sgx_orb *h) { return h ? h->g.kp_cap : SGX_ERR_INVALID; }

extern "C" int sgx_orb_get_tables(const sgx_orb *h, float *scale, float *inv_scale, float *sigma2, float *inv_sigma2, int32_t *per_level)
{
    if (!h) return SGX_ERR_INVALID;
    for (int l = 0; l < h->g.nlevels; l++) {
        if (scale) scale[l] = h->scale[l];
        if (inv_scale) inv_scale[l] = h->inv_scale[l];
        if (sigma2) sigma2[l] = h->sigma2[l];
        if (inv_sigma2) inv_sigma2[l] = h->inv_sigma2[l];
        if (per_level) per_level[l] = h->g.lv[l].quota;
    }
    return SGX_OK;
}

static void launch_octree(sgx_orb *h, int batch, sgx_stream_t stream)
{
    const SgxOrbGeom &g = h->g; const int nl = g.nlevels;
    static const int oct_threads = sgx_getenv("SGX_TUNE_OCT_THREADS") ? atoi(sgx_getenv("SGX_TUNE_OCT_THREADS")) : SGX_OCT_THREADS;
    static const bool frame_fast = sgx_getenv("SGX_TUNE_OCT_FRAME_FAST") != nullptr;
    const dim3 ogrid = frame_fast ? dim3(batch, nl) : dim3(nl, batch);
    if (h->oct_maxlim <= 256) {
        auto ka = k_octree<true, 256, 2048>; auto kb = k_octree<true, 256, SGX_CAND_LDS>; auto kc = k_octree<false, 256, 1>;
        SGX_LAUNCH(ka, ogrid, dim3(oct_threads), stream, g, h->d_cand, h->d_cand_count, h->d_node_scratch, h->d_sel, h->d_sel_count, h->d_status, -1);
        SGX_LAUNCH(kb, ogrid, dim3(oct_threads), stream, g, h->d_cand, h->d_cand_count, h->d_node_scratch, h->d_sel, h->d_sel_count, h->d_status, 2048);
        SGX_LAUNCH(kc, ogrid, dim3(oct_threads), stream, g, h->d_cand, h->d_cand_count, h->d_node_scratch, h->d_sel, h->d_sel_count, h->d_status, SGX_CAND_LDS);
    } else {
        auto kb = k_octree<true, SGX_OCT_MAXN, SGX_CAND_LDS>; auto kc = k_octree<false, SGX_OCT_MAXN, 1>;
        SGX_LAUNCH(kb, ogrid, dim3(oct_threads), stream, g, h->d_cand, h->d_cand_count, h->d_node_scratch, h->d_sel, h->d_sel_count, h->d_status, -1);
        SGX_LAUNCH(kc, ogrid, dim3(oct_threads), stream, g, h->d_cand, h->d_cand_count, h->d_node_scratch, h->d_sel, h->d_sel_count, h->d_status, SGX_CAND_LDS);
    }
}

extern "C" int sgx_orb_extract_batch_dev(sgx_orb *h, const uint8_t *d_gray, int pitch, int batch,
                                         sgx_keypoint *d_kps, uint8_t *d_desc, int32_t *d_count, int cap, void *stream_)
{
    if (!h || !d_gray || !d_kps || !d_desc || !d_count) return SGX_ERR_INVALID;
    if (batch < 1 || batch > h->cfg.max_batch || pitch < h->g.W || (pitch & 3) || ((uintptr_t)d_gray & 3) || cap < h->g.kp_cap) return SGX_ERR_INVALID;
    sgx_stream_t stream = (sgx_stream_t)stream_;
    const SgxOrbGeom &g = h->g;
    const int nl = g.nlevels;
    h->last_batch = batch;
    SGX_CHECK_HIP(hipMemsetAsync(h->d_cand_count, 0, (size_t)batch * nl * 4, stream));
    sgx_prof_begin(SGX_K_RESIZE, stream);
    static const int pyr_threads = sgx_getenv("SGX_TUNE_PYR_THREADS") ? atoi(sgx_getenv("SGX_TUNE_PYR_THREADS")) : 512;
    if (h->pyr_tiles > 0 && !g_orb_unfused_pyramid)
        SGX_LAUNCH_DYN(k_pyramid, dim3(h->pyr_tiles, batch), dim3(pyr_threads), h->pyr_lds, stream, g, h->pyr_tabs, d_gray, pitch, h->d_pyr, h->d_xt_all, h->d_yt_all, h->d_pyr_rects);
    else
        for (int l = 1; l < nl; l++) {
            dim3 grid((g.lv[l].w + 255) / 256, (g.lv[l].h + 3) / 4, batch);
            SGX_LAUNCH(k_resize, grid, dim3(256), stream, g, l, d_gray, pitch, h->d_pyr, h->d_xt[l], h->d_yt[l]);
        }
    sgx_prof_end(SGX_K_RESIZE, stream);
    sgx_prof_begin(SGX_K_FAST, stream);
    static const int fast_threads = sgx_getenv("SGX_TUNE_FAST_THREADS") ? atoi(sgx_getenv("SGX_TUNE_FAST_THREADS")) : 128;
    static const int e_extra = sgx_getenv("SGX_TUNE_E_EXTRA_LDS") ? atoi(sgx_getenv("SGX_TUNE_E_EXTRA_LDS")) : 0;
    SGX_LAUNCH_DYN(k_fast_cells, dim3(g.ncells * batch), dim3(fast_threads), g.fast_lds_bytes + e_extra, stream, g, h->d_cells, d_gray, pitch, h->d_pyr, batch,
               h->d_cand, h->d_cand_count, h->d_status);
    sgx_prof_end(SGX_K_FAST, stream);
    sgx_prof_begin(SGX_K_OCTREE, stream);
    launch_octree(h, batch, stream);
    sgx_prof_end(SGX_K_OCTREE, stream);
    sgx_prof_begin(SGX_K_ORIENT_DESC, stream);
    unsigned long long umax_packed = 0;
    for (int i = 0; i < 16; i++) umax_packed |= (unsigned long long)(h->umax_h[i] & 15) << (4 * i);
#ifdef SGX_DEBUG_TAPS
    static const bool patch_blur = sgx_getenv("SGX_TUNE_ORB_PATCH_BLUR") != nullptr;
    if (patch_blur) {
        SGX_LAUNCH_DYN(k_orient_desc, dim3(g.kp_cap * batch), dim3(64), e_extra / 2, stream, g, d_gray, pitch, h->d_pyr, h->d_sel, h->d_sel_count,
                       umax_packed, h->d_pattern, (uint8_t *)d_kps, d_desc, d_count, cap, batch, h->d_status);
    } else
#endif
    {
        static const int blur_threads = sgx_getenv("SGX_TUNE_BLUR_THREADS") ? atoi(sgx_getenv("SGX_TUNE_BLUR_THREADS")) : 256;
        {
            const int blur_grid = sgx_getenv("SGX_TUNE_ORB_BLUR_GRID") ? atoi(sgx_getenv("SGX_TUNE_ORB_BLUR_GRID")) : 4096;
            const int parts = std::min(g.nblur_tiles, std::max(1, blur_grid / batch));
            SGX_LAUNCH(k_blur_levels, dim3(parts * batch), dim3(std::min(512, std::max(256, blur_threads))), stream, g, h->d_blur_tiles, d_gray, pitch, h->d_pyr, h->d_blur, batch);
        }
#ifdef SGX_DEBUG_TAPS
        static const bool one_per_wave = sgx_getenv("SGX_TUNE_ORB_DESC_ONE_PER_WAVE") != nullptr;
        if (one_per_wave)
            SGX_LAUNCH(k_orient_desc2, dim3(g.kp_cap * batch), dim3(64), stream, g, d_gray, pitch, h->d_pyr, h->d_blur, h->d_sel, h->d_sel_count,
                       umax_packed, h->d_pattern, (uint8_t *)d_kps, d_desc, d_count, cap, batch, h->d_status);
        else
#endif
            SGX_LAUNCH(k_orient_desc4, dim3(((g.kp_cap + 3) / 4) * batch), dim3(64), stream, g, d_gray, pitch, h->d_pyr, h->d_blur, h->d_sel, h->d_sel_count,
                       umax_packed, h->d_pattern, (uint8_t *)d_kps, d_desc, d_count, cap, batch, h->d_status);
    }
    sgx_prof_end(SGX_K_ORIENT_DESC, stream);
    SGX_CHECK_HIP(hipGetLastError());
    return SGX_OK;
}

extern "C" int sgx_orb_last_status(sgx_orb *h, void *stream_)
{
    if (!h) return SGX_ERR_INVALID;
    uint32_t st = 0;
    SGX_CHECK_HIP(hipMemcpyAsync(&st, h->d_status, 4, hipMemcpyDeviceToHost, (sgx_stream_t)stream_));
    SGX_CHECK_HIP(hipStreamSynchronize((sgx_stream_t)stream_));
    if (st) { SGX_CHECK_HIP(hipMemsetAsync(h->d_status, 0, 4, (sgx_stream_t)stream_)); return SGX_ERR_OVERFLOW; }
    return SGX_OK;
}

extern "C" int sgx_orb_extract(sgx_orb *h, const uint8_t *gray, int stride, sgx_keypoint *kps, uint8_t *desc, int cap, int *n)
{
    if (!h || !gray || !kps || !desc || !n || stride < h->g.W || cap < 0) return SGX_ERR_INVALID;
    const int W = h->g.W, H = h->g.H, kc = h->g.kp_cap, P = (W + 3) & ~3;
    if (stride == P) SGX_CHECK_HIP(hipMemcpyAsync(h->d_gray1, gray, (size_t)P * (H - 1) + W, hipMemcpyHostToDevice, 0));
    else for (int y = 0; y < H; y++)
        SGX_CHECK_HIP(hipMemcpyAsync(h->d_gray1 + (size_t)y * P, gray + (size_t)y * stride, W, hipMemcpyHostToDevice, 0));
    int rc = sgx_orb_extract_batch_dev(h, h->d_gray1, P, 1, (sgx_keypoint *)h->d_kps1, h->d_desc1, h->d_count1, kc, 0);
    if (rc != SGX_OK) return rc;
    int cnt = 0;
    SGX_CHECK_HIP(hipMemcpyAsync(&cnt, h->d_count1, 4, hipMemcpyDeviceToHost, 0));
    SGX_CHECK_HIP(hipStreamSynchronize(0));
    rc = sgx_orb_last_status(h, 0);
    if (rc != SGX_OK) return rc;
    if (cnt > cap) return SGX_ERR_OVERFLOW;
    SGX_CHECK_HIP(hipMemcpyAsync(kps, h->d_kps1, (size_t)cnt * 28, hipMemcpyDeviceToHost, 0));
    SGX_CHECK_HIP(hipMemcpyAsync(desc, h->d_desc1, (size_t)cnt * 32, hipMemcpyDeviceToHost, 0));
    SGX_CHECK_HIP(hipStreamSynchronize(0));
    *n = cnt;
    return SGX_OK;
}

SGX_TAP int sgx_orb_debug_level_geometry(const sgx_orb *h, int level, int32_t *w, int32_t *hgt, int32_t *stride)
{
    if (!h || level < 0 || level >= h->g.nlevels) return SGX_ERR_INVALID;
    if (w) *w = h->g.lv[level].w; if (hgt) *hgt = h->g.lv[level].h; if (stride) *stride = h->g.lv[level].stride;
    return SGX_OK;
}

SGX_TAP int sgx_orb_debug_read_level(sgx_orb *h, int frame, int level, uint8_t *dst)
{
    if (!h || !dst || level < 1 || level >= h->g.nlevels || frame < 0 || frame >= h->cfg.max_batch) return SGX_ERR_INVALID;
    const SgxLevel &L = h->g.lv[level];
    for (int y = 0; y < L.h; y++)
        SGX_CHECK_HIP(hipMemcpyAsync(dst + (size_t)y * L.w, h->d_pyr + (size_t)frame * h->g.pyr_pitch + L.off + (size_t)y * L.stride, L.w, hipMemcpyDeviceToHost, 0));
    SGX_CHECK_HIP(hipStreamSynchronize(0));
    return SGX_OK;
}

SGX_TAP int sgx_orb_debug_read_candidates(sgx_orb *h, int frame, int level, int32_t *x, int32_t *y, int32_t *score, int cap, int *n)
{
    if (!h || !n || level < 0 || level >= h->g.nlevels || frame < 0 || frame >= h->cfg.max_batch) return SGX_ERR_INVALID;
    int cnt = 0;
    SGX_CHECK_HIP(hipMemcpyAsync(&cnt, h->d_cand_count + frame * h->g.nlevels + level, 4, hipMemcpyDeviceToHost, 0));
    SGX_CHECK_HIP(hipStreamSynchronize(0));
    if (cnt > h->g.lv[level].cand_cap) cnt = h->g.lv[level].cand_cap;
    std::vector<uint32_t> buf(cnt > 0 ? cnt : 1);
    SGX_CHECK_HIP(hipMemcpyAsync(buf.data(), h->d_cand + (size_t)frame * h->g.cand_pitch + h->g.lv[level].cand_off, (size_t)cnt * 4, hipMemcpyDeviceToHost, 0));
    SGX_CHECK_HIP(hipStreamSynchronize(0));
    for (int i = 0; i < cnt && i < cap; i++) { x[i] = buf[i] & 0xFFF; y[i] = (buf[i] >> 12) & 0xFFF; score[i] = buf[i] >> 24; }
    *n = cnt;
    return SGX_OK;
}

SGX_TAP int sgx_orb_debug_run_octree(sgx_orb *h, int level, const uint32_t *packed, int n, uint32_t *out_sel, int cap, int *nsel)
{
    if (!h || !packed || !out_sel || !nsel || level < 0 || level >= h->g.nlevels || n < 0 || n > h->g.lv[level].cand_cap) return SGX_ERR_INVALID;
    const int nl = h->g.nlevels;
    std::vector<int> cnt(nl, 0); cnt[level] = n;
    SGX_CHECK_HIP(hipMemcpyAsync(h->d_cand_count, cnt.data(), nl * 4, hipMemcpyHostToDevice, 0));
    SGX_CHECK_HIP(hipMemcpyAsync(h->d_cand + h->g.lv[level].cand_off, packed, (size_t)n * 4, hipMemcpyHostToDevice, 0));
    launch_octree(h, 1, (sgx_stream_t)0);
    int ns = 0;
    SGX_CHECK_HIP(hipMemcpyAsync(&ns, h->d_sel_count + level, 4, hipMemcpyDeviceToHost, 0));
    SGX_CHECK_HIP(hipStreamSynchronize(0));
    if (ns > cap) return SGX_ERR_OVERFLOW;
    SGX_CHECK_HIP(hipMemcpyAsync(out_sel, h->d_sel + (size_t)level * SGX_OCT_MAXN, (size_t)ns * 4, hipMemcpyDeviceToHost, 0));
    SGX_CHECK_HIP(hipStreamSynchronize(0));
    *nsel = ns;
    return sgx_orb_last_status(h, 0);
}
```

### sg_slam_amd/csrc/sgx_orb_kernels.h

```cpp
#pragma once
#include "sgx_rt.h"
#include "sgx_block.h"

#define SGX_MAX_LEVELS 12
#define SGX_EDGE 19
#define SGX_BORDER 16
#define SGX_TILE_MAX 68
#define SGX_TILE_STRIDE 72
#define SGX_CAND_LDS 8192
#define SGX_OCT_MAXN 1280
#define SGX_OCT_THREADS 512

struct SgxLevel {
    int w, h, stride;
    int off;
    int quota;
    int ncols, nrows, wcell, hcell;
    int cell0;
    int patch_size;
    int cand_off, cand_cap;
    int boff, bstride;
    float scale;
};

struct SgxOrbGeom {
    int nlevels, W, H;
    int pyr_pitch;
    int ncells;
    int kp_cap;
    int fast_off_score, fast_off_qlist, fast_off_out, fast_lds_bytes;
    int cand_pitch;
    int blur_pitch, nblur_tiles;
    int ini_th, min_th;
    SgxLevel lv[SGX_MAX_LEVELS];
};

struct SgxCell { short level, x0, y0, cw, ch, ox, oy, pad; };

#define SGX_ST_CAND_OVERFLOW 1u
#define SGX_ST_NODE_OVERFLOW 2u
#define SGX_ST_KP_OVERFLOW 4u

SGX_DEV const uint8_t *sgx_level_ptr(const SgxOrbGeom &g, const uint8_t *gray, int gray_pitch, const uint8_t *pyr,
                                     int frame, int level, int *stride)
{
    if (level == 0) { *stride = gray_pitch; return gray + (size_t)frame * gray_pitch * g.H; }
    *stride = g.lv[level].stride;
    return pyr + (size_t)frame * g.pyr_pitch + g.lv[level].off;
}

struct SgxXTab { short sx, sx1, a0, a1; };
struct SgxYTab { short sy0, sy1, b0, b1; };

SGX_KERNEL(256) k_resize(SgxOrbGeom g, int level, const uint8_t *gray, int gray_pitch, uint8_t *pyr,
                         const SgxXTab *xt, const SgxYTab *yt)
{
    SGX_THREADS_BEGIN(tid)
    const int dw = g.lv[level].w, dh = g.lv[level].h;
    const int x4 = ((int)blockIdx.x * 64 + (tid & 63)) * 4;
    const int y = (int)blockIdx.y * 4 + (tid >> 6);
    const int frame = (int)blockIdx.z;
    if (x4 < dw && y < dh) {
        int sstride, dstride;
        const uint8_t *src = sgx_level_ptr(g, gray, gray_pitch, pyr, frame, level - 1, &sstride);
        uint8_t *dst = (uint8_t *)sgx_level_ptr(g, gray, gray_pitch, pyr, frame, level, &dstride);
        const SgxYTab ty = yt[y];
        const uint8_t *r0 = src + (size_t)ty.sy0 * sstride, *r1 = src + (size_t)ty.sy1 * sstride;
        uint32_t out = 0;
#pragma unroll
        for (int i = 0; i < 4; i++) {
            const int x = x4 + i;
            if (x < dw) {
                const SgxXTab tx = xt[x];
                const int h0 = r0[tx.sx] * tx.a0 + r0[tx.sx1] * tx.a1;
                const int h1 = r1[tx.sx] * tx.a0 + r1[tx.sx1] * tx.a1;
                const int v = (((ty.b0 * (h0 >> 4)) >> 16) + ((ty.b1 * (h1 >> 4)) >> 16) + 2) >> 2;
                out |= (uint32_t)(v & 255) << (8 * i);
            }
        }
        *(uint32_t *)(dst + (size_t)y * dstride + x4) = out;
    }
    SGX_THREADS_END
}

struct SgxPyrRect { short nx0, ny0, nw, nh, ox0, oy0, ox1, oy1; unsigned qmagic; int xo, yo, pad; };
struct SgxPyrTabs { int xoff[SGX_MAX_LEVELS], yoff[SGX_MAX_LEVELS]; int lds_a, lds_b, lds_x; };

SGX_DEV unsigned sgx_udiv_magic(unsigned n, unsigned m)
{
#ifndef SGX_EMU
    return m ? __umulhi(n, m) : n;
#else
    return m ? (unsigned)(((unsigned long long)n * m) >> 32) : n;
#endif
}

SGX_KERNEL(1024) k_pyramid(SgxOrbGeom g, SgxPyrTabs tb, const uint8_t *gray, int gray_pitch, uint8_t *pyr, const SgxXTab *xt, const SgxYTab *yt,
                          const SgxPyrRect *rects)
{
    SGX_DYN_LDS(smem);
    const int tile = (int)blockIdx.x, frame = (int)blockIdx.y, nl = g.nlevels;
    const SgxPyrRect *R = rects + (size_t)tile * nl;
    uint8_t *cur = smem, *nxt = smem + tb.lds_a;
    SgxXTab *xtl_lds = (SgxXTab *)(smem + tb.lds_a + tb.lds_b); SgxYTab *ytl_lds = (SgxYTab *)(smem + tb.lds_a + tb.lds_b + tb.lds_x);
    {
        const SgxPyrRect r0 = R[0];
        const uint8_t *src = gray + (size_t)frame * gray_pitch * g.H;
        const int q = r0.nw >> 2, groups = q * r0.nh;
        SGX_THREADS_BEGIN(tid)
        for (int idx = tid; idx < groups; idx += (int)blockDim.x) {
            const int y = (int)sgx_udiv_magic((unsigned)idx, r0.qmagic), x4 = (idx - y * q) * 4;
            *(uint32_t *)(cur + y * r0.nw + x4) = *(const uint32_t *)(src + (size_t)(r0.ny0 + y) * gray_pitch + r0.nx0 + x4);
        }
        for (int l = 1; l < nl; l++) {
            const SgxPyrRect r = R[l];
            const int nx = min((int)r.nw, g.lv[l].w - r.nx0);
            for (int i = tid; i < nx; i += (int)blockDim.x) xtl_lds[r.xo + i] = xt[tb.xoff[l] + r.nx0 + i];
            for (int i = tid; i < r.nh; i += (int)blockDim.x) ytl_lds[r.yo + i] = yt[tb.yoff[l] + r.ny0 + i];
        }
        SGX_THREADS_END
    }
    SGX_SYNC();
    for (int l = 1; l < nl; l++) {
        const SgxPyrRect rp = R[l - 1], r = R[l];
        const int W = g.lv[l].w, dstride = g.lv[l].stride;
        uint8_t *dst = pyr + (size_t)frame * g.pyr_pitch + g.lv[l].off;
        const SgxXTab *xtl = xtl_lds + r.xo - r.nx0; const SgxYTab *ytl = ytl_lds + r.yo - r.ny0;
        const int q = r.nw >> 2, groups = q * r.nh;
        SGX_THREADS_BEGIN(tid)
        for (int idx = tid; idx < groups; idx += (int)blockDim.x) {
            const int y = (int)sgx_udiv_magic((unsigned)idx, r.qmagic), x4 = (idx - y * q) * 4;
            const int gy = r.ny0 + y, gx4 = r.nx0 + x4;
            const SgxYTab ty = ytl[gy];
            const uint8_t *r0 = cur + (ty.sy0 - rp.ny0) * rp.nw - rp.nx0, *r1 = cur + (ty.sy1 - rp.ny0) * rp.nw - rp.nx0;
            uint32_t out = 0;
#pragma unroll
            for (int i = 0; i < 4; i++) {
                const int x = gx4 + i;
                if (x < W) {
                    const SgxXTab tx = xtl[x];
                    const int h0 = r0[tx.sx] * tx.a0 + r0[tx.sx1] * tx.a1;
                    const int h1 = r1[tx.sx] * tx.a0 + r1[tx.sx1] * tx.a1;
                    const int v = (((ty.b0 * (h0 >> 4)) >> 16) + ((ty.b1 * (h1 >> 4)) >> 16) + 2) >> 2;
                    out |= (uint32_t)(v & 255) << (8 * i);
                }
            }
            *(uint32_t *)(nxt + y * r.nw + x4) = out;
            if (gy >= r.oy0 && gy < r.oy1 && gx4 >= r.ox0 && gx4 < r.ox1) *(uint32_t *)(dst + (size_t)gy * dstride + gx4) = out;
        }
        SGX_THREADS_END
        SGX_SYNC();
        uint8_t *t = cur; cur = nxt; nxt = t;
    }
}

SGX_DEV uint32_t sgx_alignbyte(uint32_t hi, uint32_t lo, int sh)
{
#ifndef SGX_EMU
    return __builtin_amdgcn_alignbyte(hi, lo, (uint32_t)sh);
#else
    return (uint32_t)((((unsigned long long)hi << 32) | lo) >> (8 * sh));
#endif
}

SGX_DEV uint32_t sgx_udot4(uint32_t a, uint32_t b, uint32_t c)
{
#ifndef SGX_EMU
    return __builtin_amdgcn_udot4(a, b, c, false);
#else
    for (int i = 0; i < 4; i++) c += ((a >> (8 * i)) & 255u) * ((b >> (8 * i)) & 255u);
    return c;
#endif
}
SGX_DEV uint32_t sgx_udot2(uint32_t a, uint32_t b, uint32_t c)
{
#ifndef SGX_EMU
    typedef unsigned short sgx_us2 __attribute__((ext_vector_type(2)));
    return __builtin_amdgcn_udot2(__builtin_bit_cast(sgx_us2, a), __builtin_bit_cast(sgx_us2, b), c, false);
#else
    return c + (a & 0xFFFFu) * (b & 0xFFFFu) + (a >> 16) * (b >> 16);
#endif
}

#ifndef SGX_EMU
typedef unsigned short sgx_u16x2 __attribute__((ext_vector_type(2)));
SGX_DEV uint32_t sgx_pk_usubsat_u16(uint32_t a, uint32_t b)
{
    const sgx_u16x2 r = __builtin_elementwise_sub_sat(__builtin_bit_cast(sgx_u16x2, a), __builtin_bit_cast(sgx_u16x2, b));
    return __builtin_bit_cast(uint32_t, r);
}
SGX_DEV uint32_t sgx_pk_min_u16(uint32_t a, uint32_t b)
{
    const sgx_u16x2 r = __builtin_elementwise_min(__builtin_bit_cast(sgx_u16x2, a), __builtin_bit_cast(sgx_u16x2, b));
    return __builtin_bit_cast(uint32_t, r);
}
SGX_DEV uint32_t sgx_pk_max_u16(uint32_t a, uint32_t b)
{
    const sgx_u16x2 r = __builtin_elementwise_max(__builtin_bit_cast(sgx_u16x2, a), __builtin_bit_cast(sgx_u16x2, b));
    return __builtin_bit_cast(uint32_t, r);
}
SGX_DEV uint32_t sgx_even_bytes_u16(uint32_t v) { return __builtin_amdgcn_perm(0u, v, 0x0c020c00u); }
SGX_DEV uint32_t sgx_odd_bytes_u16(uint32_t v) { return __builtin_amdgcn_perm(0u, v, 0x0c030c01u); }
#else
SGX_DEV uint32_t sgx_pk_usubsat_u16(uint32_t a, uint32_t b)
{
    const uint32_t al = a & 0xFFFFu, ah = a >> 16, bl = b & 0xFFFFu, bh = b >> 16;
    return (al > bl ? al - bl : 0u) | ((ah > bh ? ah - bh : 0u) << 16);
}
SGX_DEV uint32_t sgx_pk_min_u16(uint32_t a, uint32_t b)
{
    const uint32_t al = a & 0xFFFFu, ah = a >> 16, bl = b & 0xFFFFu, bh = b >> 16;
    return (al < bl ? al : bl) | ((ah < bh ? ah : bh) << 16);
}
SGX_DEV uint32_t sgx_pk_max_u16(uint32_t a, uint32_t b)
{
    const uint32_t al = a & 0xFFFFu, ah = a >> 16, bl = b & 0xFFFFu, bh = b >> 16;
    return (al > bl ? al : bl) | ((ah > bh ? ah : bh) << 16);
}
SGX_DEV uint32_t sgx_even_bytes_u16(uint32_t v) { return v & 0x00FF00FFu; }
SGX_DEV uint32_t sgx_odd_bytes_u16(uint32_t v) { return (v >> 8) & 0x00FF00FFu; }
#endif

SGX_DEV uint32_t sgx_alignbit(uint32_t hi, uint32_t lo, int sh)
{
#ifndef SGX_EMU
    return __builtin_amdgcn_alignbit(hi, lo, (uint32_t)sh);
#else
    return (uint32_t)((((unsigned long long)hi << 32) | lo) >> sh);
#endif
}

SGX_DEV uint32_t sgx_has9(uint32_t m16)
{
    uint32_t m = m16 | (m16 << 16);
    uint32_t a = m & (m >> 1);
    uint32_t b = a & (a >> 2);
    uint32_t c = b & (b >> 4);
    return (c & (m >> 8)) & 0xFFFFu;
}

#define SGX_FAST_THREADS 256
SGX_KERNEL(SGX_FAST_THREADS) k_fast_cells(SgxOrbGeom g, const SgxCell *cells, const uint8_t *gray, int gray_pitch, const uint8_t *pyr,
                             int batch, uint32_t *cand, int *cand_count, uint32_t *status)
{
    SGX_DYN_LDS(pool);
    uint32_t *tile_dw = (uint32_t *)pool;
    uint8_t *score = (uint8_t *)pool + g.fast_off_score;
    uint16_t *qlist = (uint16_t *)((uint8_t *)pool + g.fast_off_qlist);
    uint32_t *outbuf = (uint32_t *)((uint8_t *)pool + g.fast_off_out);
    SGX_LDS int n_lo, out_base, n_quick;
    const uint8_t *tile = (const uint8_t *)tile_dw;

    const int bid = (int)blockIdx.x;
    const int frame = bid % batch, cid = bid / batch;
    const SgxCell c = cells[cid];
    const int cw = c.cw, ch = c.ch, level = c.level;
    int stride;
    const uint8_t *img = sgx_level_ptr(g, gray, gray_pitch, pyr, frame, level, &stride);
    const int thr_lo = g.min_th, thr_hi = g.ini_th;
    const int xa = c.x0 & ~3, lead = c.x0 - xa, ndw = (lead + cw + 3) >> 2;
    const int SD = SGX_TILE_STRIDE / 4;

    SGX_THREADS_BEGIN(tid)
    if (tid == 0) { n_lo = 0; n_quick = 0; }
    for (int i = tid; i < ch * SD; i += (int)blockDim.x) {
        const int r = i / SD, q = i - r * SD;
        tile_dw[i] = q < ndw ? *(const uint32_t *)(img + (size_t)(c.y0 + r) * stride + xa + 4 * q) : 0u;
    }
    for (int i = tid; i < ch * SD; i += (int)blockDim.x) ((uint32_t *)score)[i] = 0u;
    SGX_THREADS_END
    SGX_SYNC();

    const int ih = ch - 6, ng = (lead + cw + 3) >> 2;
    const unsigned ng_m16 = (unsigned)(unsigned short)c.pad;
    for (int pass = 0; pass < 2; pass++) {
        const int thr = pass == 0 ? thr_hi : thr_lo;
        SGX_THREADS_BEGIN(tid)
        for (int t = tid; t < ih * ng; t += (int)blockDim.x) {
            const int yq = (int)(((unsigned)t * ng_m16) >> 16), y = 3 + yq, gq = t - yq * ng;
            const int x0 = 4 * gq + 3 - lead;
            if (x0 + 3 < 3 || x0 >= cw - 3) continue;
            const uint32_t *rc = tile_dw + y * SD + gq, *rp = rc + 3 * SD, *rm = rc - 3 * SD;
            const bool has1 = gq + 1 < SD, has2 = gq + 2 < SD;
            const uint32_t C0 = rc[0], C1 = has1 ? rc[1] : 0u, C2 = has2 ? rc[2] : 0u;
            const uint32_t P0 = rp[0], P1 = has1 ? rp[1] : 0u, M0 = rm[0], M1 = has1 ? rm[1] : 0u;
            const uint32_t V = sgx_alignbyte(C1, C0, 3), R4 = sgx_alignbyte(C2, C1, 2), R12 = C0, R0 = sgx_alignbyte(P1, P0, 3), R8 = sgx_alignbyte(M1, M0, 3);
            const uint32_t T2 = (uint32_t)thr * 0x00010001u;
            uint32_t any[2];
#if !defined(SGX_FAST_QUICK_V2)
    #pragma unroll
            for (int s2 = 0; s2 < 2; s2++) {
                const int sh = 8 * s2;
                const uint32_t v = (V >> sh) & 0x00FF00FFu, r0 = (R0 >> sh) & 0x00FF00FFu, r8 = (R8 >> sh) & 0x00FF00FFu, r4 = (R4 >> sh) & 0x00FF00FFu, r12 = (R12 >> sh) & 0x00FF00FFu;
                const uint32_t hi = v + T2, lo = sgx_pk_usubsat_u16(v, T2);
                const uint32_t br = sgx_pk_min_u16(sgx_pk_usubsat_u16(r0, hi) | sgx_pk_usubsat_u16(r8, hi), sgx_pk_usubsat_u16(r4, hi) | sgx_pk_usubsat_u16(r12, hi));
                const uint32_t dk = sgx_pk_min_u16(sgx_pk_usubsat_u16(lo, r0) | sgx_pk_usubsat_u16(lo, r8), sgx_pk_usubsat_u16(lo, r4) | sgx_pk_usubsat_u16(lo, r12));
                any[s2] = br | dk;
            }
#else
    #pragma unroll
            for (int s2 = 0; s2 < 2; s2++) {
                const uint32_t v = s2 ? sgx_odd_bytes_u16(V) : sgx_even_bytes_u16(V), r0 = s2 ? sgx_odd_bytes_u16(R0) : sgx_even_bytes_u16(R0), r8 = s2 ? sgx_odd_bytes_u16(R8) : sgx_even_bytes_u16(R8),
                               r4 = s2 ? sgx_odd_bytes_u16(R4) : sgx_even_bytes_u16(R4), r12 = s2 ? sgx_odd_bytes_u16(R12) : sgx_even_bytes_u16(R12);
                const uint32_t hi = v + T2, lo = sgx_pk_usubsat_u16(v, T2);
                const uint32_t br = sgx_pk_usubsat_u16(sgx_pk_min_u16(sgx_pk_max_u16(r0, r8), sgx_pk_max_u16(r4, r12)), hi);
                const uint32_t dk = sgx_pk_usubsat_u16(lo, sgx_pk_max_u16(sgx_pk_min_u16(r0, r8), sgx_pk_min_u16(r4, r12)));
                any[s2] = br | dk;
            }
#endif
            if ((any[0] | any[1]) == 0u) continue;
    #pragma unroll
            for (int i = 0; i < 4; i++) {
                const int x = x0 + i;
                const uint32_t f = (any[i & 1] >> (16 * (i >> 1))) & 0xFFFFu;
                if (x >= 3 && x < cw - 3 && f) {
                    const int slot = sgx_atomic_add(&n_quick, 1);
                    qlist[slot] = (uint16_t)(y * SGX_TILE_STRIDE + lead + x);
                }
            }
        }
        SGX_THREADS_END
        SGX_SYNC();

        SGX_THREADS_BEGIN(tid)
        for (int t = tid; t < n_quick; t += (int)blockDim.x) {
            const int pos = qlist[t];
            const uint8_t *p = tile + pos;
            const int v = p[0], lo = v - thr, hi = v + thr;
            int r[16];
            r[0] = p[3 * SGX_TILE_STRIDE];       r[1] = p[3 * SGX_TILE_STRIDE + 1];  r[2] = p[2 * SGX_TILE_STRIDE + 2];
            r[3] = p[SGX_TILE_STRIDE + 3];       r[4] = p[3];                        r[5] = p[-SGX_TILE_STRIDE + 3];
            r[6] = p[-2 * SGX_TILE_STRIDE + 2];  r[7] = p[-3 * SGX_TILE_STRIDE + 1]; r[8] = p[-3 * SGX_TILE_STRIDE];
            r[9] = p[-3 * SGX_TILE_STRIDE - 1];  r[10] = p[-2 * SGX_TILE_STRIDE - 2]; r[11] = p[-SGX_TILE_STRIDE - 3];
            r[12] = p[-3];                       r[13] = p[SGX_TILE_STRIDE - 3];     r[14] = p[2 * SGX_TILE_STRIDE - 2];
            r[15] = p[3 * SGX_TILE_STRIDE - 1];
            uint32_t mb = 0, md = 0;
    #pragma unroll
            for (int k = 0; k < 16; k++) { mb = sgx_alignbit(mb, (uint32_t)(hi - r[k]), 31); md = sgx_alignbit(md, (uint32_t)(r[k] - lo), 31); }
            if (!(sgx_has9(mb & 0xFFFFu) | sgx_has9(md & 0xFFFFu))) continue;
            qlist[t] = (uint16_t)(pos | 0x8000);
            int d[16];
    #pragma unroll
            for (int k = 0; k < 16; k++) d[k] = v - r[k];
            int mn2[16], mx2[16], mn4[16], mx4[16];
    #pragma unroll
            for (int k = 0; k < 16; k++) { mn2[k] = min(d[k], d[(k + 1) & 15]); mx2[k] = max(d[k], d[(k + 1) & 15]); }
    #pragma unroll
            for (int k = 0; k < 16; k++) { mn4[k] = min(mn2[k], mn2[(k + 2) & 15]); mx4[k] = max(mx2[k], mx2[(k + 2) & 15]); }
            int A = -512, Bm = 512;
    #pragma unroll
            for (int k = 0; k < 16; k++) {
                const int mn9 = min(min(mn4[k], mn4[(k + 4) & 15]), d[(k + 8) & 15]);
                const int mx9 = max(max(mx4[k], mx4[(k + 4) & 15]), d[(k + 8) & 15]);
                A = max(A, mn9); Bm = min(Bm, mx9);
            }
            const int s = max(A, -Bm) - 1;
            score[pos] = (uint8_t)s;
        }
        SGX_THREADS_END
        SGX_SYNC();

        SGX_THREADS_BEGIN(tid)
        for (int i = tid; i < n_quick; i += (int)blockDim.x) {
            if (!(qlist[i] & 0x8000)) continue;
            const int pos = qlist[i] & 0x7FFF;
            const uint8_t *s = score + pos;
            const int v = s[0];
            const bool mx = v > s[-1] && v > s[1] && v > s[-SGX_TILE_STRIDE - 1] && v > s[-SGX_TILE_STRIDE] && v > s[-SGX_TILE_STRIDE + 1] &&
                            v > s[SGX_TILE_STRIDE - 1] && v > s[SGX_TILE_STRIDE] && v > s[SGX_TILE_STRIDE + 1];
            if (mx && v >= thr) {
                const int slot = sgx_atomic_add(&n_lo, 1);
                const int y = pos / SGX_TILE_STRIDE, x = pos - y * SGX_TILE_STRIDE - lead;
                outbuf[slot] = (uint32_t)(x + c.ox) | ((uint32_t)(y + c.oy) << 12) | ((uint32_t)v << 24);
            }
        }
        SGX_THREADS_END
        SGX_SYNC();

        if (n_lo > 0 || thr_hi == thr_lo) break;
        SGX_THREADS_BEGIN(tid) if (tid == 0) n_quick = 0; SGX_THREADS_END
        SGX_SYNC();
    }

    const int n_emit = n_lo;
    SGX_THREADS_BEGIN(tid)
    if (tid == 0 && n_emit > 0) out_base = sgx_atomic_add(&cand_count[frame * g.nlevels + level], n_emit);
    SGX_THREADS_END
    SGX_SYNC();
    if (n_emit > 0) {
        uint32_t *dst = cand + (size_t)frame * g.cand_pitch + g.lv[level].cand_off;
        const int dcap = g.lv[level].cand_cap;
        SGX_THREADS_BEGIN(tid)
        for (int i = tid; i < n_emit; i += (int)blockDim.x) {
            const int slot = out_base + i;
            if (slot < dcap) dst[slot] = outbuf[i];
            else sgx_atomic_or(status, SGX_ST_CAND_OVERFLOW);
        }
        SGX_THREADS_END
    }
}


struct SgxOctNode { uint16_t ulx, uly, urx, bry; };

SGX_DEV int sgx_oct_quadrant(const SgxOctNode b, uint32_t e)
{
    const int halfX = (int)ceilf((float)(b.urx - b.ulx) / 2), halfY = (int)ceilf((float)(b.bry - b.uly) / 2);
    const float x = (float)(e & 0xFFF), y = (float)((e >> 12) & 0xFFF);
    const float sx = (float)(b.ulx + halfX), sy = (float)(b.uly + halfY);
    return (x < sx) ? ((y < sy) ? 0 : 2) : ((y < sy) ? 1 : 3);
}

SGX_DEV unsigned long long sgx_oct_pick_key(uint32_t e, int wcell, int hcell)
{
    const int x = (int)(e & 0xFFF), y = (int)((e >> 12) & 0xFFF);
    const int cj = (x - 3) / wcell, ci = (y - 3) / hcell;
    const unsigned long long rank = ((unsigned long long)ci << 30) | ((unsigned long long)cj << 20) |
                                    ((unsigned long long)(y - ci * hcell) << 10) | (unsigned long long)(x - cj * wcell);
    return ((unsigned long long)(e >> 24) << 40) | (0xFFFFFFFFFFull - rank);
}

template <bool KEYS_IN_LDS, int MAXN, int CL>
SGX_KERNEL(512) k_octree(SgxOrbGeom g, const uint32_t *cand, const int *cand_count, uint16_t *node_scratch,
                                     uint32_t *sel, int *sel_count, uint32_t *status, int nk_lo)
{
    SGX_LDS uint32_t kxy_lds[KEYS_IN_LDS ? CL : 1];
    SGX_LDS uint16_t node_lds[KEYS_IN_LDS ? CL : 1];
    SGX_LDS SgxOctNode nb[2][MAXN];
    SGX_LDS uint16_t ncnt[2][MAXN];
    SGX_LDS uint16_t nseq[2][MAXN];
    SGX_LDS uint8_t nflag[2][MAXN];
    SGX_LDS int quad[MAXN][4];
    SGX_LDS int scanA[MAXN];
    SGX_LDS int scanB[MAXN];
    SGX_LDS uint8_t splitting[MAXN];
    SGX_LDS uint16_t order[MAXN];
    SGX_LDS uint16_t rank_of[MAXN];
    SGX_LDS unsigned long long best[MAXN];
    SGX_LDS int s_size, s_C, s_kept, s_ntoexpand, s_stop, s_m, s_overflow;

    const bool frames_fast = (int)gridDim.y == g.nlevels;
    const int frame = (int)(frames_fast ? blockIdx.x : blockIdx.y), level = (int)(frames_fast ? blockIdx.y : blockIdx.x);
    const SgxLevel L = g.lv[level];
    const int N = L.quota;
    int nk = cand_count[frame * g.nlevels + level];
    if (nk > L.cand_cap) nk = L.cand_cap;
    if (nk <= nk_lo || (KEYS_IN_LDS && nk > CL)) return;
    const uint32_t *src = cand + (size_t)frame * g.cand_pitch + L.cand_off;
    uint32_t *kxy = KEYS_IN_LDS ? kxy_lds : (uint32_t *)src;
    uint16_t *node_of = KEYS_IN_LDS ? node_lds : node_scratch + (size_t)frame * g.cand_pitch + L.cand_off;
    uint32_t *out = sel + ((size_t)frame * g.nlevels + level) * SGX_OCT_MAXN;
    const int NT = (int)blockDim.x;

    const int minX = SGX_BORDER, maxX = L.w - SGX_EDGE + 3, minY = SGX_BORDER, maxY = L.h - SGX_EDGE + 3;
    const int nIni = (int)roundf((float)(maxX - minX) / (float)(maxY - minY));
    const float hX = nIni > 0 ? (float)(maxX - minX) / (float)nIni : 1.f;

    if (nk == 0 || nIni < 1 || nIni > 64) {
        SGX_THREADS_BEGIN(tid) if (tid == 0) sel_count[frame * g.nlevels + level] = 0; SGX_THREADS_END
        return;
    }

    SGX_THREADS_BEGIN(tid)
    for (int i = tid; i < nIni; i += NT) scanA[i] = 0;
    if (tid == 0) s_overflow = 0;
    SGX_THREADS_END
    SGX_SYNC();
    SGX_THREADS_BEGIN(tid)
    for (int k = tid; k < nk; k += NT) {
        const uint32_t e = src[k];
        if (KEYS_IN_LDS) kxy[k] = e;
        const int r = (int)((float)(e & 0xFFF) / hX);
        node_of[k] = (uint16_t)r;
        sgx_atomic_add(&scanA[r], 1);
    }
    SGX_THREADS_END
    SGX_SYNC();
    SGX_THREADS_BEGIN(tid)
    if (tid == 0) {
        int n = 0;
        for (int i = 0; i < nIni; i++) {
            const int c = scanA[i];
            if (c == 0) { scanB[i] = -1; continue; }
            nb[0][n].ulx = (uint16_t)(int)(hX * (float)i); nb[0][n].uly = 0;
// ... 732 lines not shown
```

### sg_slam_amd/flow.py

```python
import ctypes as C
import numpy as np
from .capi import FlowConfig, _vp
from ._lib import load


class OpticalFlowLK:

    def __init__(self, width=640, height=480, max_batch=1, win_size=21, max_level=3, max_count=30, epsilon=0.01, lib=None):
        self.lib = lib if lib is not None else load()
        self.cfg = FlowConfig(width, height, max_batch, win_size, max_level, max_count, epsilon)
        h = C.c_void_p()
        self.lib.check(self.lib.dll.sgx_flow_create(C.byref(self.cfg), C.byref(h)), 'sgx_flow_create')
        self.h = h
        self.width, self.height, self.max_batch = width, height, max_batch
        self.levels = self.lib.dll.sgx_flow_levels(self.h)

    def close(self):
        if getattr(self, 'h', None):
            self.lib.dll.sgx_flow_destroy(self.h)
            self.h = None

    def __del__(self):
        try:
            self.close()
        except Exception:
            pass

    def reset(self):
        self.lib.check(self.lib.dll.sgx_flow_reset(self.h), 'sgx_flow_reset')

    def __call__(self, gray_from, gray_to, pts):
        a = np.ascontiguousarray(gray_from, np.uint8); b = np.ascontiguousarray(gray_to, np.uint8)
        assert a.shape == b.shape == (self.height, self.width)
        p = np.ascontiguousarray(pts, 'f4').reshape(-1, 2); n = len(p)
        out = np.zeros((max(n, 1), 2), 'f4'); st = np.zeros(max(n, 1), np.uint8)
        self.lib.check(self.lib.dll.sgx_flow_lk(self.h, _vp(a), _vp(b), self.width, _vp(p), n, _vp(out), _vp(st)), 'sgx_flow_lk')
        return out[:n], st[:n]

    def lk_batch_dev(self, d_gray, pitch, batch, d_keys, d_n, cap, d_prev_xy, d_status=None, stream=None):
        have = C.c_int32(0)
        self.lib.check(self.lib.dll.sgx_flow_lk_batch_dev(self.h, _vp(d_gray), pitch, batch, _vp(d_keys), _vp(d_n), cap, _vp(d_prev_xy), _vp(d_status),
                                                          C.byref(have), _vp(stream)), 'sgx_flow_lk_batch_dev')
        return bool(have.value)

    def debug_level(self, slot, frame, level):
        w, h = C.c_int32(), C.c_int32()
        self.lib.check(self.lib.tap('sgx_flow_debug_level_size')(self.h, level, C.byref(w), C.byref(h)))
        img = np.zeros((h.value, w.value), np.uint8)
        self.lib.check(self.lib.tap('sgx_flow_debug_read_level')(self.h, slot, frame, level, _vp(img)), 'flow debug_read_level')
        return img


def find_fundamental_mat(pts1, pts2, threshold=1.0, confidence=0.99, lib=None):
    lib = lib if lib is not None else load()
    a = np.ascontiguousarray(pts1, 'f4').reshape(-1, 2); b = np.ascontiguousarray(pts2, 'f4').reshape(-1, 2)
    assert len(a) == len(b)
    F = np.zeros(9, 'f8'); ok = np.zeros(1, 'i4'); stats = np.zeros(4, 'i4')
    lib.check(lib.dll.sgx_find_fundamental_mat(_vp(a), _vp(b), len(a), threshold, confidence, _vp(F), _vp(ok), _vp(stats)), 'sgx_find_fundamental_mat')
    return int(ok[0]), F.reshape(3, 3), stats


def fundamental_ransac_batch_dev(lib, batch, cap, d_keys, d_n, d_prev_xy, d_F, d_ok, d_stats=None, pre_have=None, pre_boxes=None, pre_nboxes=None, max_boxes=0,
                                 threshold=1.0, confidence=0.99, stream=None):
    lib.check(lib.dll.sgx_fundamental_ransac_batch_dev(batch, cap, _vp(d_keys), _vp(d_n), _vp(d_prev_xy), _vp(pre_have), _vp(pre_boxes), _vp(pre_nboxes), max_boxes,
                                                       threshold, confidence, _vp(d_F), _vp(d_ok), _vp(d_stats), _vp(stream)), 'sgx_fundamental_ransac_batch_dev')
```

Measured before the change: 29560.

## Fuse LK pyramid copy with first downsample and rework ORB pyramid resize

The LK flow pyramid no longer runs a separate copy kernel followed by one pyrdown launch per level. The copy is fused into the first downsample, and each thread now produces two output rows using udot4/alignbyte byte arithmetic with separate plain and border paths. All remaining levels run in a single per-frame 1024-thread tail kernel. The ORB resize pyramid switches to per-4-pixel x-groups using perm and udot2 and reuses horizontally filtered rows across vertical segments, which removes the LDS x-table staging. This cuts launches and per-pixel instruction count, but adds complexity, and the tail kernel uses only one block per frame, which limits parallelism.

Measured after the change: 30000, median of 6. 1.5% higher.

```diff
diff --git a/include/sgx_debug.h b/include/sgx_debug.h
--- a/include/sgx_debug.h
+++ b/include/sgx_debug.h
@@ -18,6 +18,7 @@
 int sgx_ba_debug_set_solver(int mode);
 int sgx_det_debug_read_blob(sgx_det *h, const char *blob_name, int image, float *dst, int cap, int *n);
 int sgx_flow_debug_read_level(sgx_flow *h, int slot, int frame, int level, uint8_t *img);
+int sgx_flow_debug_read_slot(sgx_flow *h, int slot, int frame, int level, uint8_t *img, int32_t *pitch);
 int sgx_flow_debug_level_size(const sgx_flow *h, int level, int32_t *w, int32_t *hgt);
 int sgx_pnp_debug_betas(int which, const double *L, const double *rho, double *betas);
 int sgx_debug_corun_bf16(int blocks, int iters, int launches, void *stream);
diff --git a/sg_slam_amd/capi.py b/sg_slam_amd/capi.py
--- a/sg_slam_amd/capi.py
+++ b/sg_slam_amd/capi.py
@@ -87,7 +87,7 @@
     'sgx_orb_debug_run_octree', 'sgx_pose_opt_debug_set_threads', 'sgx_ba_debug_set_solver', 'sgx_ba_debug_set_jobs', 'sgx_ba_debug_set_init', 'sgx_ba_debug_last_plan', 'sgx_det_debug_read_blob',
     'sgx_det_debug_detection_output', 'sgx_det_debug_continued', 'sgx_debug_flow_affine_batch_dev', 'sgx_det_debug_set_fusion', 'sgx_det_debug_set_legacy_kernels',
     'sgx_det_debug_set_block_fusion', 'sgx_det_debug_set_irb', 'sgx_det_debug_set_gemm', 'sgx_det_debug_time_ops', 'sgx_det_debug_run_step', 'sgx_flow_debug_read_level',
-    'sgx_flow_debug_level_size', 'sgx_debug_corun_bf16', 'sgx_pnp_debug_betas',
+    'sgx_flow_debug_level_size', 'sgx_flow_debug_read_slot', 'sgx_debug_corun_bf16', 'sgx_pnp_debug_betas',
 ]
 
 
@@ -246,6 +246,7 @@
             d.sgx_debug_corun_bf16.argtypes = [C.c_int, C.c_int, C.c_int, vp]
             d.sgx_pnp_debug_betas.argtypes = [C.c_int, vp, vp, vp]
             d.sgx_flow_debug_level_size.argtypes = [vp, C.c_int, C.POINTER(C.c_int32), C.POINTER(C.c_int32)]
+            d.sgx_flow_debug_read_slot.argtypes = [vp, C.c_int, C.c_int, C.c_int, vp, C.POINTER(C.c_int32)]
 
     def tap(self, name):
         if not self.has_taps:
diff --git a/sg_slam_amd/csrc/sgx_flow.cpp b/sg_slam_amd/csrc/sgx_flow.cpp
--- a/sg_slam_amd/csrc/sgx_flow.cpp
+++ b/sg_slam_amd/csrc/sgx_flow.cpp
@@ -9,6 +9,7 @@
 #include <stdlib.h>
 #include <string.h>
 #include <new>
+#include <algorithm>
 #include <vector>
 
 
@@ -66,10 +67,20 @@
     uint8_t *base = h->img[slot];
     sgx_prof_begin(SGX_K_LK_PYR, st);
     auto magic = [](int d) -> unsigned { return d <= 1 ? 0u : (unsigned)((0x100000000ull + (unsigned)d - 1) / (unsigned)d); };
-    SGX_LAUNCH(k_lk_copy, dim3(((g.pitch[0] >> 2) * g.h[0] + 255) / 256, batch), dim3(256), st, d_gray, g.w[0], g.h[0], pitch, base, g.pitch[0], g.img_stride, magic(g.pitch[0] >> 2));
-    for (int l = 1; l < g.nl; l++)
-        SGX_LAUNCH(k_lk_pyrdown, dim3(((g.pitch[l] >> 2) * g.h[l] + 255) / 256, batch), dim3(256), st, (const uint8_t *)(base + g.ioff[l - 1]), g.w[l - 1], g.h[l - 1], g.pitch[l - 1],
-                   g.img_stride, base + g.ioff[l], g.w[l], g.h[l], g.pitch[l], g.img_stride, magic(g.pitch[l] >> 2));
+    if (g.nl == 1)
+        SGX_LAUNCH(k_lk_copy, dim3(((g.pitch[0] >> 2) * g.h[0] + 255) / 256, batch), dim3(256), st, d_gray, g.w[0], g.h[0], pitch, base, g.pitch[0], g.img_stride, magic(g.pitch[0] >> 2));
+    else {
+        SgxLkDiv dv;
+        memset(&dv, 0, sizeof dv);
+        for (int l = 1; l < g.nl; l++) {
+            const int sw = g.w[l - 1], sp = l == 1 ? pitch : g.pitch[l - 1], qw = g.pitch[l] >> 2;
+            const int gf = std::max(1, std::min(qw, std::min((sw - 9) >> 3, (sp - 12) >> 3) + 1));
+            dv.gf[l] = gf; dv.plain[l] = magic(gf - 1); dv.border[l] = magic(qw - gf + 1);
+        }
+        const int nrp = (g.h[1] + 1) >> 1, plain_blocks = ((dv.gf[1] - 1) * nrp + 255) / 256, border_blocks = (((g.pitch[1] >> 2) - dv.gf[1] + 1) * nrp + 255) / 256;
+        SGX_LAUNCH(k_lk_pyr01, dim3(plain_blocks + border_blocks, batch), dim3(256), st, d_gray, pitch, g, base, dv, plain_blocks);
+        if (g.nl > 2) SGX_LAUNCH(k_lk_pyrtail, dim3(batch), dim3(1024), st, g, base, dv);
+    }
     sgx_prof_end(SGX_K_LK_PYR, st);
     SGX_CHECK_HIP(hipGetLastError());
     return SGX_OK;
@@ -150,6 +161,16 @@
     }
     return SGX_OK;
 }
+SGX_TAP int sgx_flow_debug_read_slot(sgx_flow *h, int slot, int frame, int level, uint8_t *img , int32_t *pitch)
+{
+    if (!h || slot < 0 || slot > 1 || frame < 0 || frame >= h->cfg.max_batch || level < 0 || level >= h->g.nl || !pitch) return SGX_ERR_INVALID;
+    const SgxLkGeom &g = h->g;
+    *pitch = g.pitch[level];
+    if (!img) return SGX_OK;
+    SGX_CHECK_HIP(hipDeviceSynchronize());
+    SGX_CHECK_HIP(hipMemcpy(img, h->img[slot] + (size_t)frame * g.img_stride + g.ioff[level], (size_t)g.pitch[level] * g.h[level], hipMemcpyDeviceToHost));
+    return SGX_OK;
+}
 SGX_TAP int sgx_flow_debug_level_size(const sgx_flow *h, int level, int32_t *w, int32_t *hh)
 {
     if (!h || level < 0 || level >= h->g.nl || !w || !hh) return SGX_ERR_INVALID;
diff --git a/sg_slam_amd/csrc/sgx_flow_kernels.h b/sg_slam_amd/csrc/sgx_flow_kernels.h
--- a/sg_slam_amd/csrc/sgx_flow_kernels.h
+++ b/sg_slam_amd/csrc/sgx_flow_kernels.h
@@ -1,6 +1,7 @@
 #pragma once
 #include "sgx_rt.h"
 #include "sgx_block.h"
+#include "sgx_lane.h"
 #include <float.h>
 #include <math.h>
 
@@ -50,40 +51,88 @@
     SGX_THREADS_END
 }
 
-SGX_KERNEL(256) k_lk_pyrdown(const uint8_t *src, int sw, int sh, int spitch, unsigned sstride, uint8_t *dst, int dw, int dh, int dpitch, unsigned dstride, unsigned qw_magic)
+SGX_DEV int sgx_lk_reflect(int p, int len) { p = p < 0 ? -p : p; return p >= len ? 2 * len - 2 - p : p; }
+template <bool COPY, bool FAST>
+SGX_DEV void sgx_lk_down_task(const uint8_t *S, int sw, int sh, int spitch, uint8_t *D, int dh, int dpitch, uint8_t *C, int cpitch, int yp, int G)
+{
+    const int X = 4 * G, y0 = 2 * yp;
+    uint32_t acc[2][4];
+#pragma unroll
+    for (int o = 0; o < 4; o++) acc[0][o] = acc[1][o] = 128u;
+    int xi[11]; uint32_t keep[2] = { ~0u, ~0u };
+    if (!FAST) {
+#pragma unroll
+        for (int i = 0; i < 11; i++) xi[i] = sgx_lk_reflect(2 * X - 2 + i, sw);
+#pragma unroll
+        for (int i = 0; i < 8; i++) if (2 * X + i >= sw) keep[i >> 2] &= ~(0xFFu << (8 * (i & 3)));
+    }
+#pragma unroll
+    for (int k = 0; k < 7; k++) {
+        const int r = 2 * y0 - 2 + k;
+        const uint8_t *row = S + (size_t)sgx_lk_reflect(r, sh) * spitch;
+        uint32_t v[4];
+        if (FAST) __builtin_memcpy(v, row + 2 * X - 4, 16);
+        else {
+            v[0] = ((uint32_t)row[xi[0]] << 16) | ((uint32_t)row[xi[1]] << 24); v[3] = row[xi[10]];
+#pragma unroll
+            for (int j = 1; j < 3; j++) v[j] = (uint32_t)row[xi[4 * j - 2]] | ((uint32_t)row[xi[4 * j - 1]] << 8) | ((uint32_t)row[xi[4 * j]] << 16) | ((uint32_t)row[xi[4 * j + 1]] << 24);
+        }
+        const uint32_t W[6] = { sgx_alignbyte(v[1], v[0], 2), v[1], sgx_alignbyte(v[2], v[1], 2), v[2], sgx_alignbyte(v[3], v[2], 2), v[3] };
+#pragma unroll
+        for (int j = 0; j < 2; j++) {
+            const int kk = k - 2 * j;
+            if (kk < 0 || kk > 4) continue;
+            const uint32_t wk = kk == 0 || kk == 4 ? 1u : kk == 2 ? 6u : 4u;
+#pragma unroll
+            for (int o = 0; o < 4; o++) acc[j][o] = sgx_udot4(W[o + 2], wk, sgx_udot4(W[o], wk * 0x04060401u, acc[j][o]));
+        }
+        if (COPY && k >= 2 && k <= 5 && r < sh) {
+            uint8_t *c = C + (size_t)r * cpitch + 2 * X;
+            if (FAST || 2 * X < cpitch) *(uint32_t *)c = v[1] & keep[0];
+            if (FAST || 2 * X + 4 < cpitch) *(uint32_t *)(c + 4) = v[2] & keep[1];
+        }
+    }
+#pragma unroll
+    for (int j = 0; j < 2; j++)
+        if (y0 + j < dh) *(uint32_t *)(D + (size_t)(y0 + j) * dpitch + X) = sgx_perm(acc[j][1], acc[j][0], 0x0c0c0501u) | sgx_perm(acc[j][3], acc[j][2], 0x05010c0cu);
+}
+template <bool COPY>
+SGX_DEV void sgx_lk_down(int q, int nplain, int ntasks, int gf, int qw, unsigned m_plain, unsigned m_border,
+                         const uint8_t *S, int sw, int sh, int spitch, uint8_t *D, int dh, int dpitch, uint8_t *C, int cpitch)
+{
+    if (q < nplain) {
+        const int yp = (int)sgx_lk_udiv((unsigned)q, m_plain), G = 1 + q - yp * (gf - 1);
+        sgx_lk_down_task<COPY, true>(S, sw, sh, spitch, D, dh, dpitch, C, cpitch, yp, G);
+    } else if (q < ntasks) {
+        const int e = q - nplain, nb = qw - gf + 1, yp = (int)sgx_lk_udiv((unsigned)e, m_border), i = e - yp * nb;
+        sgx_lk_down_task<COPY, false>(S, sw, sh, spitch, D, dh, dpitch, C, cpitch, yp, i == 0 ? 0 : gf + i - 1);
+    }
+}
+struct SgxLkDiv { int gf[SGX_LK_MAXL]; unsigned plain[SGX_LK_MAXL], border[SGX_LK_MAXL]; };
+
+SGX_KERNEL(256) k_lk_pyr01(const uint8_t *src, int spitch, SgxLkGeom g, uint8_t *base, SgxLkDiv dv, int plain_blocks)
 {
     SGX_THREADS_BEGIN(tid)
-    const int f = (int)blockIdx.y, qw = dpitch >> 2, q = (int)blockIdx.x * 256 + tid;
-    if (q < qw * dh) {
-        const int y = (int)sgx_lk_udiv((unsigned)q, qw_magic), X = (q - y * qw) * 4;
-        const uint8_t *S = src + (size_t)f * sstride;
-        int acc[4] = { 0, 0, 0, 0 };
-        const bool fast = X >= 2 && 2 * X + 11 < spitch && 2 * X + 8 <= sw - 1;
-#pragma unroll
-        for (int k = 0; k < 5; k++) {
-            const int wk = k == 0 || k == 4 ? 1 : k == 2 ? 6 : 4;
-            const uint8_t *row = S + (size_t)sgx_reflect101(2 * y - 2 + k, sh) * spitch;
-            int p[11];
-            if (fast) {
-                const uint32_t *r4 = (const uint32_t *)(row + 2 * X - 4);
-                const uint32_t a = r4[0], b = r4[1], c = r4[2], d = r4[3];
-                p[0] = (a >> 16) & 255; p[1] = a >> 24;
-                p[2] = b & 255; p[3] = (b >> 8) & 255; p[4] = (b >> 16) & 255; p[5] = b >> 24;
-                p[6] = c & 255; p[7] = (c >> 8) & 255; p[8] = (c >> 16) & 255; p[9] = c >> 24;
-                p[10] = d & 255;
-            } else {
-#pragma unroll
-                for (int i = 0; i < 11; i++) p[i] = row[sgx_reflect101(2 * X - 2 + i, sw)];
-            }
-#pragma unroll
-            for (int o = 0; o < 4; o++) acc[o] += wk * (p[2 * o + 2] * 6 + (p[2 * o + 1] + p[2 * o + 3]) * 4 + p[2 * o] + p[2 * o + 4]);
-        }
-        uint32_t out = 0;
-#pragma unroll
-        for (int o = 0; o < 4; o++) out |= (uint32_t)((acc[o] + 128) >> 8) << (8 * o);
-        *(uint32_t *)(dst + (size_t)f * dstride + (size_t)y * dpitch + X) = out;
-    }
+    const int f = (int)blockIdx.y, qw = g.pitch[1] >> 2, nrp = (g.h[1] + 1) >> 1, gf = dv.gf[1];
+    const int nplain = (gf - 1) * nrp, ntasks = qw * nrp;
+    const int q = (int)blockIdx.x < plain_blocks ? min((int)blockIdx.x * 256 + tid, nplain) : nplain + ((int)blockIdx.x - plain_blocks) * 256 + tid;
+    uint8_t *img = base + (size_t)f * g.img_stride;
+    if ((int)blockIdx.x >= plain_blocks || q < nplain)
+        sgx_lk_down<true>(q, nplain, ntasks, gf, qw, dv.plain[1], dv.border[1], src + (size_t)f * g.h[0] * spitch, g.w[0], g.h[0], spitch, img + g.ioff[1], g.h[1], g.pitch[1], img, g.pitch[0]);
     SGX_THREADS_END
+}
+SGX_KERNEL(1024) k_lk_pyrtail(SgxLkGeom g, uint8_t *base, SgxLkDiv dv)
+{
+    uint8_t *img = base + (size_t)blockIdx.x * g.img_stride;
+    for (int l = 2; l < g.nl; l++) {
+        const int qw = g.pitch[l] >> 2, nrp = (g.h[l] + 1) >> 1, gf = dv.gf[l];
+        const int nplain = (gf - 1) * nrp, ntasks = qw * nrp;
+        SGX_THREADS_BEGIN(tid)
+        for (int q = tid; q < ntasks; q += (int)blockDim.x)
+            sgx_lk_down<false>(q, nplain, ntasks, gf, qw, dv.plain[l], dv.border[l], img + g.ioff[l - 1], g.w[l - 1], g.h[l - 1], g.pitch[l - 1], img + g.ioff[l], g.h[l], g.pitch[l], nullptr, 0);
+        SGX_THREADS_END
+        SGX_SYNC();
+    }
 }
 
 struct SgxLkWeights { int w00, w01, w10, w11; };
diff --git a/sg_slam_amd/csrc/sgx_lane.h b/sg_slam_amd/csrc/sgx_lane.h
--- /dev/null
+++ b/sg_slam_amd/csrc/sgx_lane.h
@@ -0,0 +1,51 @@
+#pragma once
+#include "sgx_rt.h"
+
+SGX_DEV uint32_t sgx_alignbyte(uint32_t hi, uint32_t lo, int sh)
+{
+#ifndef SGX_EMU
+    return __builtin_amdgcn_alignbyte(hi, lo, (uint32_t)sh);
+#else
+    return (uint32_t)((((unsigned long long)hi << 32) | lo) >> (8 * sh));
+#endif
+}
+
+SGX_DEV uint32_t sgx_udot4(uint32_t a, uint32_t b, uint32_t c)
+{
+#ifndef SGX_EMU
+    return __builtin_amdgcn_udot4(a, b, c, false);
+#else
+    for (int i = 0; i < 4; i++) c += ((a >> (8 * i)) & 255u) * ((b >> (8 * i)) & 255u);
+    return c;
+#endif
+}
+SGX_DEV uint32_t sgx_udot2(uint32_t a, uint32_t b, uint32_t c)
+{
+#ifndef SGX_EMU
+    typedef unsigned short sgx_us2 __attribute__((ext_vector_type(2)));
+    return __builtin_amdgcn_udot2(__builtin_bit_cast(sgx_us2, a), __builtin_bit_cast(sgx_us2, b), c, false);
+#else
+    return c + (a & 0xFFFFu) * (b & 0xFFFFu) + (a >> 16) * (b >> 16);
+#endif
+}
+
+SGX_DEV uint32_t sgx_perm(uint32_t hi, uint32_t lo, uint32_t sel)
+{
+#ifndef SGX_EMU
+    return __builtin_amdgcn_perm(hi, lo, sel);
+#else
+    const unsigned long long v = ((unsigned long long)hi << 32) | lo;
+    uint32_t r = 0;
+    for (int i = 0; i < 4; i++) { const uint32_t s = (sel >> (8 * i)) & 255u; if (s < 8u) r |= (uint32_t)((v >> (8 * s)) & 255u) << (8 * i); }
+    return r;
+#endif
+}
+
+SGX_DEV uint32_t sgx_umul24(uint32_t a, uint32_t b)
+{
+#ifndef SGX_EMU
+    return __umul24(a, b);
+#else
+    return a * b;
+#endif
+}
diff --git a/sg_slam_amd/csrc/sgx_orb.cpp b/sg_slam_amd/csrc/sgx_orb.cpp
--- a/sg_slam_amd/csrc/sgx_orb.cpp
+++ b/sg_slam_amd/csrc/sgx_orb.cpp
@@ -24,7 +24,7 @@
     SgxCell *d_cells = nullptr;
     SgxXTab *d_xt[SGX_MAX_LEVELS] = {};
     SgxYTab *d_yt[SGX_MAX_LEVELS] = {};
-    SgxXTab *d_xt_all = nullptr; SgxYTab *d_yt_all = nullptr; SgxPyrRect *d_pyr_rects = nullptr; SgxPyrTabs pyr_tabs; int pyr_tiles = 0, pyr_lds = 0;
+    SgxXGroup *d_xg_all = nullptr; SgxYTab *d_yt_all = nullptr; SgxPyrRect *d_pyr_rects = nullptr; SgxPyrTabs pyr_tabs; int pyr_tiles = 0, pyr_lds = 0;
     int *d_umax = nullptr;
     signed char *d_pattern = nullptr;
     uint8_t *d_pyr = nullptr;
@@ -120,7 +120,7 @@
     (void)hipFree(h->d_cand_count); (void)hipFree(h->d_node_scratch); (void)hipFree(h->d_sel); (void)hipFree(h->d_sel_count); (void)hipFree(h->d_status);
     (void)hipFree(h->d_gray1); (void)hipFree(h->d_kps1); (void)hipFree(h->d_desc1); (void)hipFree(h->d_count1);
     for (int l = 0; l < SGX_MAX_LEVELS; l++) { (void)hipFree(h->d_xt[l]); (void)hipFree(h->d_yt[l]); }
-    (void)hipFree(h->d_xt_all); (void)hipFree(h->d_yt_all); (void)hipFree(h->d_pyr_rects); (void)hipFree(h->d_blur); (void)hipFree(h->d_blur_tiles);
+    (void)hipFree(h->d_xg_all); (void)hipFree(h->d_yt_all); (void)hipFree(h->d_pyr_rects); (void)hipFree(h->d_blur); (void)hipFree(h->d_blur_tiles);
     delete h;
 }
 
@@ -245,16 +245,31 @@
     SGX_CHECK_HIP(hipStreamSynchronize(0));
     if (nl > 1) {
         std::vector<std::vector<SgxXTab>> xts(nl); std::vector<std::vector<SgxYTab>> yts(nl);
-        std::vector<SgxXTab> xall; std::vector<SgxYTab> yall;
+        std::vector<SgxXGroup> xall; std::vector<SgxYTab> yall;
+        bool span_ok = true;
         memset(&h->pyr_tabs, 0, sizeof h->pyr_tabs);
         for (int l = 1; l < nl; l++) {
             build_resize_tables(g.lv[l - 1].w, g.lv[l - 1].h, g.lv[l].w, g.lv[l].h, xts[l], yts[l]);
             h->pyr_tabs.xoff[l] = (int)xall.size(); h->pyr_tabs.yoff[l] = (int)yall.size();
-            xall.insert(xall.end(), xts[l].begin(), xts[l].end()); yall.insert(yall.end(), yts[l].begin(), yts[l].end());
+            yall.insert(yall.end(), yts[l].begin(), yts[l].end());
+            for (int x4 = 0; x4 < g.lv[l].w; x4 += 4) {
+                SgxXGroup G; memset(&G, 0, sizeof G);
+                G.sx0 = xts[l][x4].sx;
+                for (int i = 0; i < 4; i++) {
+                    G.sel[i] = 0x0c0c0c0cu;
+                    if (x4 + i >= g.lv[l].w) continue;
+                    const SgxXTab &t = xts[l][x4 + i];
+                    const int o0 = t.sx - G.sx0, o1 = t.sx1 - G.sx0;
+                    if (o0 < 0 || o1 < 0 || o0 >= SGX_PYR_SPAN || o1 >= SGX_PYR_SPAN || t.a0 < 0 || t.a1 < 0) { span_ok = false; continue; }
+                    G.sel[i] = (uint32_t)o0 | 0x0c00u | ((uint32_t)o1 << 16) | 0x0c000000u;
+                    G.a01[i] = (uint32_t)t.a0 | ((uint32_t)t.a1 << 16);
+                }
+                xall.push_back(G);
+            }
         }
         const int T = 32, ntx = (g.lv[nl - 1].w + T - 1) / T, nty = (g.lv[nl - 1].h + T - 1) / T;
         std::vector<SgxPyrRect> rects((size_t)ntx * nty * nl);
-        int max_a = 0, max_b = 0, max_x = 0, max_y = 0;
+        int max_a = 0, max_b = 0, max_y = 0;
         for (int j = 0; j < nty; j++) for (int i = 0; i < ntx; i++) {
             SgxPyrRect *R = &rects[((size_t)j * ntx + i) * nl];
             int nx0 = 0, nx1 = 0, ny0 = 0, ny1 = 0;
@@ -273,22 +288,22 @@
                 }
                 ax0 &= ~3; ax1 = (ax1 + 3) & ~3;
                 r.nx0 = (short)ax0; r.ny0 = (short)ay0; r.nw = (short)(ax1 - ax0); r.nh = (short)(ay1 - ay0);
-                const int q = r.nw / 4; r.qmagic = q <= 1 ? 0u : (unsigned)((0x100000000ull + (unsigned)q - 1) / (unsigned)q); r.pad = 0;
+                const int q = r.nw / 4; r.qmagic = q <= 1 ? 0u : (unsigned)((0x100000000ull + (unsigned)q - 1) / (unsigned)q); r.pad0 = r.pad1 = 0;
                 const int bytes = (int)r.nw * r.nh;
                 if (l & 1) max_b = std::max(max_b, bytes); else max_a = std::max(max_a, bytes);
                 nx0 = ax0; nx1 = ax1; ny0 = ay0; ny1 = ay1;
             }
-            int xo = 0, yo = 0;
-            for (int l = 1; l < nl; l++) { R[l].xo = xo; R[l].yo = yo; xo += R[l].nw; yo += R[l].nh; }
-            R[0].xo = R[0].yo = 0;
-            max_x = std::max(max_x, xo); max_y = std::max(max_y, yo);
-        }
-        h->pyr_tabs.lds_a = (max_a + 15) & ~15; h->pyr_tabs.lds_b = (max_b + 15) & ~15; h->pyr_tabs.lds_x = max_x * (int)sizeof(SgxXTab);
-        h->pyr_lds = h->pyr_tabs.lds_a + h->pyr_tabs.lds_b + h->pyr_tabs.lds_x + max_y * (int)sizeof(SgxYTab);
+            int yo = 0;
+            for (int l = 1; l < nl; l++) { R[l].yo = yo; yo += R[l].nh; }
+            R[0].yo = 0;
+            max_y = std::max(max_y, yo);
+        }
+        h->pyr_tabs.lds_a = (max_a + SGX_PYR_SPAN + 15) & ~15; h->pyr_tabs.lds_b = (max_b + SGX_PYR_SPAN + 15) & ~15;
+        h->pyr_lds = h->pyr_tabs.lds_a + h->pyr_tabs.lds_b + max_y * (int)sizeof(SgxYTab);
         h->pyr_tiles = ntx * nty;
-        if (h->pyr_lds > 64 * 1024) h->pyr_tiles = 0;
-        SGX_ALLOC(h->d_xt_all, xall.size() * sizeof(SgxXTab)); SGX_ALLOC(h->d_yt_all, yall.size() * sizeof(SgxYTab)); SGX_ALLOC(h->d_pyr_rects, rects.size() * sizeof(SgxPyrRect));
-        SGX_CHECK_HIP(hipMemcpy(h->d_xt_all, xall.data(), xall.size() * sizeof(SgxXTab), hipMemcpyHostToDevice));
+        if (h->pyr_lds > 64 * 1024 || !span_ok) h->pyr_tiles = 0;
+        SGX_ALLOC(h->d_xg_all, xall.size() * sizeof(SgxXGroup)); SGX_ALLOC(h->d_yt_all, yall.size() * sizeof(SgxYTab)); SGX_ALLOC(h->d_pyr_rects, rects.size() * sizeof(SgxPyrRect));
+        SGX_CHECK_HIP(hipMemcpy(h->d_xg_all, xall.data(), xall.size() * sizeof(SgxXGroup), hipMemcpyHostToDevice));
         SGX_CHECK_HIP(hipMemcpy(h->d_yt_all, yall.data(), yall.size() * sizeof(SgxYTab), hipMemcpyHostToDevice));
         SGX_CHECK_HIP(hipMemcpy(h->d_pyr_rects, rects.data(), rects.size() * sizeof(SgxPyrRect), hipMemcpyHostToDevice));
     }
@@ -343,7 +358,7 @@
     sgx_prof_begin(SGX_K_RESIZE, stream);
     static const int pyr_threads = sgx_getenv("SGX_TUNE_PYR_THREADS") ? atoi(sgx_getenv("SGX_TUNE_PYR_THREADS")) : 512;
     if (h->pyr_tiles > 0 && !g_orb_unfused_pyramid)
-        SGX_LAUNCH_DYN(k_pyramid, dim3(h->pyr_tiles, batch), dim3(pyr_threads), h->pyr_lds, stream, g, h->pyr_tabs, d_gray, pitch, h->d_pyr, h->d_xt_all, h->d_yt_all, h->d_pyr_rects);
+        SGX_LAUNCH_DYN(k_pyramid, dim3(h->pyr_tiles, batch), dim3(pyr_threads), h->pyr_lds, stream, g, h->pyr_tabs, d_gray, pitch, h->d_pyr, h->d_xg_all, h->d_yt_all, h->d_pyr_rects);
     else
         for (int l = 1; l < nl; l++) {
             dim3 grid((g.lv[l].w + 255) / 256, (g.lv[l].h + 3) / 4, batch);
diff --git a/sg_slam_amd/csrc/sgx_orb_kernels.h b/sg_slam_amd/csrc/sgx_orb_kernels.h
--- a/sg_slam_amd/csrc/sgx_orb_kernels.h
+++ b/sg_slam_amd/csrc/sgx_orb_kernels.h
@@ -1,6 +1,7 @@
 #pragma once
 #include "sgx_rt.h"
 #include "sgx_block.h"
+#include "sgx_lane.h"
 
 #define SGX_MAX_LEVELS 12
 #define SGX_EDGE 19
@@ -83,8 +84,10 @@
     SGX_THREADS_END
 }
 
-struct SgxPyrRect { short nx0, ny0, nw, nh, ox0, oy0, ox1, oy1; unsigned qmagic; int xo, yo, pad; };
-struct SgxPyrTabs { int xoff[SGX_MAX_LEVELS], yoff[SGX_MAX_LEVELS]; int lds_a, lds_b, lds_x; };
+struct SgxPyrRect { short nx0, ny0, nw, nh, ox0, oy0, ox1, oy1; unsigned qmagic; int yo, pad0, pad1; };
+struct SgxPyrTabs { int xoff[SGX_MAX_LEVELS], yoff[SGX_MAX_LEVELS]; int lds_a, lds_b; };
+struct SgxXGroup { int sx0; uint32_t sel[4], a01[4]; };
+#define SGX_PYR_SPAN 8
 
 SGX_DEV unsigned sgx_udiv_magic(unsigned n, unsigned m)
 {
@@ -94,15 +97,22 @@
     return m ? (unsigned)(((unsigned long long)n * m) >> 32) : n;
 #endif
 }
-
-SGX_KERNEL(1024) k_pyramid(SgxOrbGeom g, SgxPyrTabs tb, const uint8_t *gray, int gray_pitch, uint8_t *pyr, const SgxXTab *xt, const SgxYTab *yt,
+SGX_DEV void sgx_pyr_hrow(const uint8_t *row, const SgxXGroup &xg, uint32_t (&H)[4])
+{
+    uint32_t w[2];
+    __builtin_memcpy(w, row, SGX_PYR_SPAN);
+#pragma unroll
+    for (int i = 0; i < 4; i++) H[i] = sgx_udot2(sgx_perm(w[1], w[0], xg.sel[i]), xg.a01[i], 0u) >> 4;
+}
+
+SGX_KERNEL(1024) k_pyramid(SgxOrbGeom g, SgxPyrTabs tb, const uint8_t *gray, int gray_pitch, uint8_t *pyr, const SgxXGroup *xg, const SgxYTab *yt,
                           const SgxPyrRect *rects)
 {
     SGX_DYN_LDS(smem);
     const int tile = (int)blockIdx.x, frame = (int)blockIdx.y, nl = g.nlevels;
     const SgxPyrRect *R = rects + (size_t)tile * nl;
     uint8_t *cur = smem, *nxt = smem + tb.lds_a;
-    SgxXTab *xtl_lds = (SgxXTab *)(smem + tb.lds_a + tb.lds_b); SgxYTab *ytl_lds = (SgxYTab *)(smem + tb.lds_a + tb.lds_b + tb.lds_x);
+    SgxYTab *ytl_lds = (SgxYTab *)(smem + tb.lds_a + tb.lds_b);
     {
         const SgxPyrRect r0 = R[0];
         const uint8_t *src = gray + (size_t)frame * gray_pitch * g.H;
@@ -114,8 +124,6 @@
         }
         for (int l = 1; l < nl; l++) {
             const SgxPyrRect r = R[l];
-            const int nx = min((int)r.nw, g.lv[l].w - r.nx0);
-            for (int i = tid; i < nx; i += (int)blockDim.x) xtl_lds[r.xo + i] = xt[tb.xoff[l] + r.nx0 + i];
             for (int i = tid; i < r.nh; i += (int)blockDim.x) ytl_lds[r.yo + i] = yt[tb.yoff[l] + r.ny0 + i];
         }
         SGX_THREADS_END
@@ -123,63 +131,40 @@
     SGX_SYNC();
     for (int l = 1; l < nl; l++) {
         const SgxPyrRect rp = R[l - 1], r = R[l];
-        const int W = g.lv[l].w, dstride = g.lv[l].stride;
+        const int dstride = g.lv[l].stride;
         uint8_t *dst = pyr + (size_t)frame * g.pyr_pitch + g.lv[l].off;
-        const SgxXTab *xtl = xtl_lds + r.xo - r.nx0; const SgxYTab *ytl = ytl_lds + r.yo - r.ny0;
-        const int q = r.nw >> 2, groups = q * r.nh;
-        SGX_THREADS_BEGIN(tid)
-        for (int idx = tid; idx < groups; idx += (int)blockDim.x) {
-            const int y = (int)sgx_udiv_magic((unsigned)idx, r.qmagic), x4 = (idx - y * q) * 4;
-            const int gy = r.ny0 + y, gx4 = r.nx0 + x4;
-            const SgxYTab ty = ytl[gy];
-            const uint8_t *r0 = cur + (ty.sy0 - rp.ny0) * rp.nw - rp.nx0, *r1 = cur + (ty.sy1 - rp.ny0) * rp.nw - rp.nx0;
-            uint32_t out = 0;
-#pragma unroll
-            for (int i = 0; i < 4; i++) {
-                const int x = gx4 + i;
-                if (x < W) {
-                    const SgxXTab tx = xtl[x];
-                    const int h0 = r0[tx.sx] * tx.a0 + r0[tx.sx1] * tx.a1;
-                    const int h1 = r1[tx.sx] * tx.a0 + r1[tx.sx1] * tx.a1;
-                    const int v = (((ty.b0 * (h0 >> 4)) >> 16) + ((ty.b1 * (h1 >> 4)) >> 16) + 2) >> 2;
-                    out |= (uint32_t)(v & 255) << (8 * i);
-                }
-            }
-            *(uint32_t *)(nxt + y * r.nw + x4) = out;
-            if (gy >= r.oy0 && gy < r.oy1 && gx4 >= r.ox0 && gx4 < r.ox1) *(uint32_t *)(dst + (size_t)gy * dstride + gx4) = out;
+        const SgxYTab *ytl = ytl_lds + r.yo;
+        const SgxXGroup *xgl = xg + tb.xoff[l] + (r.nx0 >> 2);
+        const int q = r.nw >> 2, nseg = q > 0 ? max(1, min((int)r.nh, (int)blockDim.x / q)) : 1, rs = (r.nh + nseg - 1) / nseg, tasks = q * nseg;
+        SGX_THREADS_BEGIN(tid)
+        for (int t = tid; t < tasks; t += (int)blockDim.x) {
+            const int sg = (int)sgx_udiv_magic((unsigned)t, r.qmagic), c = t - sg * q, x4 = 4 * c, gx4 = r.nx0 + x4;
+            const SgxXGroup xc = xgl[c];
+            const uint8_t *col = cur + (xc.sx0 - rp.nx0);
+            const bool own_x = gx4 >= r.ox0 && gx4 < r.ox1;
+            uint32_t HA[4], HB[4] = { 0, 0, 0, 0 }; int rowB = -1;
+            const int y1 = min(sg * rs + rs, (int)r.nh);
+            for (int y = sg * rs; y < y1; y++) {
+                const int gy = r.ny0 + y;
+                const SgxYTab ty = ytl[y];
+                const int s0 = ty.sy0 - rp.ny0, s1 = ty.sy1 - rp.ny0;
+                if (s0 == rowB) { HA[0] = HB[0]; HA[1] = HB[1]; HA[2] = HB[2]; HA[3] = HB[3]; }
+                else sgx_pyr_hrow(col + s0 * rp.nw, xc, HA);
+                if (s1 == s0) { HB[0] = HA[0]; HB[1] = HA[1]; HB[2] = HA[2]; HB[3] = HA[3]; }
+                else sgx_pyr_hrow(col + s1 * rp.nw, xc, HB);
+                rowB = s1;
+                uint32_t v[4];
+#pragma unroll
+                for (int i = 0; i < 4; i++) v[i] = ((sgx_umul24((uint32_t)ty.b0, HA[i]) >> 16) + (sgx_umul24((uint32_t)ty.b1, HB[i]) >> 16) + 2u) >> 2;
+                const uint32_t out = v[0] | (v[1] << 8) | (v[2] << 16) | (v[3] << 24);
+                *(uint32_t *)(nxt + y * r.nw + x4) = out;
+                if (own_x && gy >= r.oy0 && gy < r.oy1) *(uint32_t *)(dst + (size_t)gy * dstride + gx4) = out;
+            }
         }
         SGX_THREADS_END
         SGX_SYNC();
         uint8_t *t = cur; cur = nxt; nxt = t;
     }
-}
-
-SGX_DEV uint32_t sgx_alignbyte(uint32_t hi, uint32_t lo, int sh)
-{
-#ifndef SGX_EMU
-    return __builtin_amdgcn_alignbyte(hi, lo, (uint32_t)sh);
-#else
-    return (uint32_t)((((unsigned long long)hi << 32) | lo) >> (8 * sh));
-#endif
-}
-
-SGX_DEV uint32_t sgx_udot4(uint32_t a, uint32_t b, uint32_t c)
-{
-#ifndef SGX_EMU
-    return __builtin_amdgcn_udot4(a, b, c, false);
-#else
-    for (int i = 0; i < 4; i++) c += ((a >> (8 * i)) & 255u) * ((b >> (8 * i)) & 255u);
-    return c;
-#endif
-}
-SGX_DEV uint32_t sgx_udot2(uint32_t a, uint32_t b, uint32_t c)
-{
-#ifndef SGX_EMU
-    typedef unsigned short sgx_us2 __attribute__((ext_vector_type(2)));
-    return __builtin_amdgcn_udot2(__builtin_bit_cast(sgx_us2, a), __builtin_bit_cast(sgx_us2, b), c, false);
-#else
-    return c + (a & 0xFFFFu) * (b & 0xFFFFu) + (a >> 16) * (b >> 16);
-#endif
 }
 
 #ifndef SGX_EMU
diff --git a/sg_slam_amd/flow.py b/sg_slam_amd/flow.py
--- a/sg_slam_amd/flow.py
+++ b/sg_slam_amd/flow.py
@@ -50,6 +50,14 @@
         self.lib.check(self.lib.tap('sgx_flow_debug_read_level')(self.h, slot, frame, level, _vp(img)), 'flow debug_read_level')
         return img
 
+    def debug_slot(self, slot, frame, level):
+        w, h, p = C.c_int32(), C.c_int32(), C.c_int32()
+        self.lib.check(self.lib.tap('sgx_flow_debug_level_size')(self.h, level, C.byref(w), C.byref(h)))
+        self.lib.check(self.lib.tap('sgx_flow_debug_read_slot')(self.h, slot, frame, level, None, C.byref(p)))
+        img = np.zeros((h.value, p.value), np.uint8)
+        self.lib.check(self.lib.tap('sgx_flow_debug_read_slot')(self.h, slot, frame, level, _vp(img), C.byref(p)), 'flow debug_read_slot')
+        return img
+
 
 def find_fundamental_mat(pts1, pts2, threshold=1.0, confidence=0.99, lib=None):
     lib = lib if lib is not None else load()
```
